# amankhullar/MMBiDAF

Hardware: NVIDIA B200
Metric: mmbidaf_train_videos_per_s (higher is better)
Workload: dtype bf16 tcgen05 BiDAF + tf32 library GEMMs, fp32 accumulate / soft-max / LSTM

## Files before the change

### mmbidaf_b200/csrc/bidaf_bwd_tc.cu

```cuda
#include <stdlib.h>
#include "tc_common.cuh"

namespace mmb {
using namespace tc;
namespace {

constexpr int TY = 32;
constexpr int Y_PART = TY / 8 * GROUP_BYTES;
constexpr int MAX_STAGES = 3;
constexpr int COL_S = 0, COL_GA = 32, COL_GB = 64, COL_ACC0 = 96, COL_ACC1 = 96 + DPAD;
constexpr int STG_STRIDE = 204;
constexpr int NTHREADS = 256;
constexpr int PART_STRIDE = 3 * DPAD;
constexpr float NEG2 = kNegFill * LOG2E;

enum Mode { PT = 0, DC = 1, DQ = 2 };

__device__ __forceinline__ void l2_prefetch(const void* p, size_t bytes) {
  const uintptr_t lo = (reinterpret_cast<uintptr_t>(p) + 15) & ~uintptr_t(15), hi = (reinterpret_cast<uintptr_t>(p) + bytes) & ~uintptr_t(15);
  if (hi > lo) asm volatile("cp.async.bulk.prefetch.L2.global [%0], %1;" ::"l"(lo), "r"((uint32_t)(hi - lo)) : "memory");
}

struct PrepArgs {
  const float* grad;
  const float* text;
  const float* out;
  const float* bm;
  __nv_bfloat16* da_pack;
  __nv_bfloat16* dbm_pack;
  float* d_text;
  float* d_row;
  int L, LP, d;
};

constexpr int PACK_CHUNK_STRIDE = 144;

__device__ __forceinline__ void ld8(const float* p, float* v) {
  const float4 a = __ldg(reinterpret_cast<const float4*>(p)), b = __ldg(reinterpret_cast<const float4*>(p + 4));
  v[0] = a.x; v[1] = a.y; v[2] = a.z; v[3] = a.w; v[4] = b.x; v[5] = b.y; v[6] = b.z; v[7] = b.w;
}

__global__ void __launch_bounds__(256) bidaf_bwd_prep_kernel(const PrepArgs a) {
  __shared__ __align__(16) unsigned char stage[8][CHUNKS * PACK_CHUNK_STRIDE];
  const int b = blockIdx.y, warp = threadIdx.x >> 5, lane = threadIdx.x & 31;
  const int g = blockIdx.x * 8 + warp;
  const int d = a.d, nchunk = d >> 3;
  uint4 da_out[8], dbm_out[8];
#pragma unroll
  for (int r = 0; r < 8; ++r) {
    const int row = g * 8 + r;
    da_out[r] = dbm_out[r] = make_uint4(0u, 0u, 0u, 0u);
    float dot = 0.f;
    const bool on = row < a.L && lane < nchunk;
    if (on) {
      const size_t r4 = ((size_t)b * a.L + row) * 4 * d + lane * 8, r1 = ((size_t)b * a.L + row) * d + lane * 8;
      float g0[8], g1[8], g2[8], g3[8], c[8], av[8], bv[8];
      ld8(a.grad + r4, g0); ld8(a.grad + r4 + d, g1); ld8(a.grad + r4 + 2 * d, g2); ld8(a.grad + r4 + 3 * d, g3);
      ld8(a.text + r1, c); ld8(a.out + r4 + d, av); ld8(a.bm + r1, bv);
      float da[8], db[8], dc[8];
#pragma unroll
      for (int e = 0; e < 8; ++e) {
        da[e] = fmaf(c[e], g2[e], g1[e]);
        db[e] = c[e] * g3[e];
        dc[e] = fmaf(bv[e], g3[e], fmaf(av[e], g2[e], g0[e]));
        dot = fmaf(da[e], av[e], fmaf(db[e], bv[e], dot));
      }
      *reinterpret_cast<float4*>(a.d_text + r1) = make_float4(dc[0], dc[1], dc[2], dc[3]);
      *reinterpret_cast<float4*>(a.d_text + r1 + 4) = make_float4(dc[4], dc[5], dc[6], dc[7]);
      __nv_bfloat162 pa[4], pb[4];
#pragma unroll
      for (int e = 0; e < 4; ++e) {
        pa[e] = __floats2bfloat162_rn(da[2 * e], da[2 * e + 1]);
        pb[e] = __floats2bfloat162_rn(db[2 * e], db[2 * e + 1]);
      }
      da_out[r] = *reinterpret_cast<uint4*>(pa);
      dbm_out[r] = *reinterpret_cast<uint4*>(pb);
    }
    dot = warp_sum(dot);
    if (lane == 0 && row < a.L) a.d_row[(size_t)b * a.L + row] = dot;
  }
  unsigned char* buf = stage[warp];
  const size_t base = ((size_t)b * (a.LP / 8) + g) * GROUP_BYTES;
#pragma unroll 1
  for (int which = 0; which < 2; ++which) {
    if (lane < CHUNKS) {
#pragma unroll
      for (int r = 0; r < 8; ++r)
        *reinterpret_cast<uint4*>(buf + lane * PACK_CHUNK_STRIDE + r * 16) = which == 0 ? da_out[r] : dbm_out[r];
    }
    __syncwarp();
    uint4* dst = reinterpret_cast<uint4*>(reinterpret_cast<char*>(which == 0 ? a.da_pack : a.dbm_pack) + base);
    for (int i = lane; i < CHUNKS * 8; i += 32)
      dst[i] = *reinterpret_cast<const uint4*>(buf + (i >> 3) * PACK_CHUNK_STRIDE + (i & 7) * 16);
    __syncwarp();
  }
}

struct BwdArgs {
  const __nv_bfloat16* x_ops[4];
  const __nv_bfloat16* y_ops[4];
  const unsigned long long* x_words;
  const unsigned long long* y_words;
  const float* bias;
  const float* norm_x;
  const float* norm_y;
  const float* dlt_x;
  const float* dlt_y;
  const float* x_feat;
  const uint8_t* x_keep;
  const float* w_term;
  const float* w_fold;
  const float* t_feat;
  float* dx;
  __nv_bfloat16* dt_pack;
  float* d_col;
  float* part;
  long long* trace;
  float keep_scale;
  int LX, LXP, LY, LYP, d;
  int prefetch;
};

template <int MODE>
__device__ __forceinline__ void bwd_block(const BwdArgs& a, const int b, const int xblk, const int nxb, int* ready,
                                          const int ready_target) {
  constexpr bool IS_PT = MODE == PT;
  constexpr int ROWS = IS_PT ? 128 : 64;
  constexpr int NX = IS_PT ? 1 : 4, NY = IS_PT ? 3 : 4;
  constexpr int X_BYTES = ROWS / 8 * GROUP_BYTES;
  constexpr int TILE_BYTES = ROWS * TY * 2;
  constexpr int TILE_LBO = ROWS * 16;
  constexpr int STAGE_BYTES = NY * Y_PART;
  constexpr int HALF = TY / 2;
  constexpr int STAGES = IS_PT ? 3 : 2;
  extern __shared__ __align__(128) unsigned char smem[];
  unsigned char* Xs = smem;
  unsigned char* Ts = Xs + NX * X_BYTES;
  unsigned char* St = Ts + 2 * TILE_BYTES;
  float* ycol = reinterpret_cast<float*>(St + STAGES * STAGE_BYTES);
  uint64_t* bars = reinterpret_cast<uint64_t*>(ycol + 2 * 3 * TY);
  uint32_t* tmem_slot = reinterpret_cast<uint32_t*>(bars + 2 + 2 * MAX_STAGES);

  const int tid = threadIdx.x, warp = tid >> 5, lane = tid & 31;
  const int half = warp >> 2, wq = warp & 3;
  constexpr int MMA_M = IS_PT ? 128 : 64;
  const int row = IS_PT ? wq * 32 + lane : wq * 16 + (lane & 15);
  const bool owner = IS_PT || lane < 16;
  constexpr int MMA_WARP = IS_PT ? 0 : 2, TMA_WARP = IS_PT ? 1 : 3;
  const int warp_u = uniform_warp_idx();
  const uint32_t leader = elect_one();
  const int x0 = xblk * ROWS;
  if (x0 >= a.LX) return;
  const uint32_t bar_x = smem_u32(bars), bar_mma = smem_u32(bars + 1), bar_full0 = smem_u32(bars + 2);
  const uint32_t bar_free0 = smem_u32(bars + 2 + MAX_STAGES);

  if (tid == 0) {
    mbar_init(bar_x, 1);
    for (int s = 0; s < STAGES; ++s) {
      mbar_init(bar_full0 + 8 * s, 1);
      mbar_init(bar_free0 + 8 * s, 1);
    }
    mbar_init(bar_mma, 1);
    fence_barrier_init();
  }
  if (warp == 0) tmem_alloc(smem_u32(tmem_slot), TMEM_COLS);

  int nty = (a.LY + TY - 1) / TY;
  if (MODE == DC) {
    int last = 0;
    for (int w = lane; w < (a.LY + 63) / 64; w += 32) {
      const unsigned long long open = a.y_words[((size_t)b * (a.LYP / 64) + w) * 2 + 1];
      if (open != 0ull) last = 2 * w + ((open >> 32) != 0ull ? 2 : 1);
    }
#pragma unroll
    for (int o = 16; o > 0; o >>= 1) last = max(last, __shfl_xor_sync(0xffffffffu, last, o));
    if (last > 0) nty = min(nty, last);
  }
  const size_t x_off = ((size_t)b * (a.LXP / 8) + x0 / 8) * GROUP_BYTES;
  const size_t y_batch = (size_t)b * (a.LYP / 8) * GROUP_BYTES;
  if (a.prefetch && tid == 32 * 5) {
    const size_t e0 = ((size_t)b * a.LX + x0) * a.d, ne = (size_t)min(ROWS, a.LX - x0) * a.d;
    if (IS_PT) {
      l2_prefetch(a.t_feat + e0, ne * 4);
    } else {
      l2_prefetch(a.x_feat + e0, ne * 4);
      l2_prefetch(a.dx + e0, ne * 4);
      if (a.x_keep) l2_prefetch(a.x_keep + e0, ne);
    }
  }
  const float log2_lx = log2f((float)a.LX);
  const int yl = tid - (IS_PT ? 0 : 6 * 32);
  float yl_lse = 0.f, yl_d2 = 0.f;
  auto fetch_ycol = [&](int t) {
    const int y = t * TY + yl;
    if ((unsigned)yl < (unsigned)TY && y < a.LY) {
      yl_lse = a.norm_y[(size_t)b * a.LY + y];
      if (!IS_PT) yl_d2 = a.dlt_y[(size_t)b * a.LY + y];
    }
  };
  auto store_ycol = [&](int t) {
    if ((unsigned)yl < (unsigned)TY) {
      float n2 = 0.f, d2 = 0.f, fill = NEG2;
      if (t * TY + yl < a.LY) {
        const bool degenerate = yl_lse < -5e29f;
        n2 = degenerate ? log2_lx : yl_lse * LOG2E;
        fill = degenerate ? 0.f : NEG2;
        d2 = yl_d2;
      }
      float* yc = ycol + (t & 1) * 3 * TY;
      yc[yl] = n2;
      yc[TY + yl] = d2;
      yc[2 * TY + yl] = fill;
    }
  };
  if (!IS_PT && ready) {
    if (tid == 0) wait_counter(ready + b, ready_target);
    __syncthreads();
    fence_proxy_async_all();
  }
  fetch_ycol(0);
  store_ycol(0);
  tc_fence_before();
  __syncthreads();
  tc_fence_after();
  const uint32_t tmem = __shfl_sync(0xffffffffu, *tmem_slot, 0);

  auto issue_stage = [&](int t) {
    const int s = t % STAGES;
    const uint32_t bar = bar_full0 + 8 * s;
    const uint32_t dst = smem_u32(St + s * STAGE_BYTES);
    const size_t off = y_batch + (size_t)t * Y_PART;
    mbar_expect_tx(bar, STAGE_BYTES, leader);
#pragma unroll
    for (int p = 0; p < NY; ++p)
      tma_bulk_g2s(dst + p * Y_PART, reinterpret_cast<const char*>(a.y_ops[p]) + off, Y_PART, bar, leader);
  };
  if (warp_u == TMA_WARP) {
    mbar_expect_tx(bar_x, NX * X_BYTES, leader);
#pragma unroll
    for (int p = 0; p < NX; ++p)
      tma_bulk_g2s(smem_u32(Xs + p * X_BYTES), reinterpret_cast<const char*>(a.x_ops[p]) + x_off, X_BYTES, bar_x, leader);
    for (int t = 0; t < STAGES && t < nty; ++t) issue_stage(t);
  }

  const float bias2 = a.bias[0] * LOG2E;
  const int gx = x0 + row;
  bool valid_x = false, open_x = false;
  float n1 = 0.f, d1 = 0.f;
  if (owner) {
    const ulonglong2 xw = *reinterpret_cast<const ulonglong2*>(a.x_words + ((size_t)b * (a.LXP / 64) + gx / 64) * 2);
    valid_x = (xw.x >> (gx & 63)) & 1ull;
    open_x = (xw.y >> (gx & 63)) & 1ull;
    if (!IS_PT && valid_x) {
      n1 = a.norm_x[(size_t)b * a.LX + gx] * LOG2E;
      d1 = a.dlt_x[(size_t)b * a.LX + gx];
    }
  }
  const uint32_t lane_base = tmem + ((uint32_t)(wq * 32) << 16);
  uint32_t mma_phase = 0;
  float rsum = 0.f;
  constexpr uint32_t IDESC_S = idesc_bf16(TY, 0, MMA_M), IDESC_PV = idesc_bf16(DPAD, 1, MMA_M);
  const uint32_t xs_lo = desc_lo(smem_u32(Xs), 128), ts_lo = desc_lo(smem_u32(Ts), TILE_LBO);

  const bool tracing = a.trace != nullptr && b == 0 && xblk == 0 && tid == MMA_WARP * 32;
  int ntrace = 0;
  auto stamp = [&]() {
    if (tracing && ntrace < 250) a.trace[ntrace++] = clock64();
  };
  stamp();
  if (warp_u == MMA_WARP) mbar_wait(bar_x, 0);
  stamp();
  for (int t = 0; t < nty; ++t) {
    const int s = t % STAGES;
    const uint32_t st_addr = smem_u32(St + s * STAGE_BYTES);
    if (warp_u == MMA_WARP) {
      mbar_wait(bar_full0 + 8 * s, (t / STAGES) & 1);
      stamp();
      tc_fence_after();
      const uint32_t st_lo = desc_lo(st_addr, 128);
      constexpr int NPROD = IS_PT ? 1 : 4;
#pragma unroll
      for (int p = 0; p < NPROD; ++p) {
        const int col = p == 0 ? COL_S : p == 1 ? COL_GA : p == 3 ? COL_GB : (MODE == DC ? COL_GA : COL_GB);
        const bool fresh = p == 0 || p == 1 || (p == 2 && MODE == DQ) || (p == 3 && MODE == DC);
#pragma unroll
        for (int k = 0; k < DPAD / 16; ++k)
          umma_bf16_lh(tmem + col, xs_lo + (p * X_BYTES + k * 256) / 16, desc_hi(GROUP_BYTES),
                       st_lo + (p * Y_PART + k * 256) / 16, desc_hi(GROUP_BYTES), IDESC_S, !(fresh && k == 0), leader);
      }
      umma_commit(bar_mma, leader);
      stamp();
    }
    const ulonglong2 words = *reinterpret_cast<const ulonglong2*>(a.y_words + ((size_t)b * (a.LYP / 64) + (t >> 1)) * 2);
    const int sh = (t & 1) * 32 + half * HALF;
    const uint32_t wvalid = (uint32_t)(words.x >> sh) & 0xffffu, wopen = (uint32_t)(words.y >> sh) & 0xffffu;
    if (t + 1 < nty) fetch_ycol(t + 1);
    if (warp_u == TMA_WARP && t >= 1 && t - 1 + STAGES < nty) {
      mbar_wait(bar_free0 + 8 * ((t - 1) % STAGES), ((t - 1) / STAGES) & 1);
      issue_stage(t - 1 + STAGES);
    }
    mbar_wait(bar_mma, mma_phase);
    mma_phase ^= 1;
    tc_fence_after();
    stamp();

    {
      const float* yc = ycol + (t & 1) * 3 * TY + half * HALF;
      float sv[HALF];
      tmem_ld16(lane_base + COL_S + half * HALF, sv);
      uint32_t pk0[HALF / 2], pk1[HALF / 2];
      if (IS_PT) {
        float n2[HALF];
#pragma unroll
        for (int c = 0; c < HALF; c += 4) *reinterpret_cast<float4*>(n2 + c) = *reinterpret_cast<const float4*>(yc + c);
        const bool masked_row = __any_sync(0xffffffffu, valid_x && !open_x);
#pragma unroll
        for (int c = 0; c < HALF; c += 2) {
          float w[2];
#pragma unroll
          for (int e = 0; e < 2; ++e) {
            float logit = fmaf(sv[c + e], LOG2E, bias2);
            if (masked_row && !open_x) logit = yc[2 * TY + c + e];
            w[e] = (valid_x && ((wvalid >> (c + e)) & 1u)) ? fast_exp2(logit - n2[c + e]) : 0.f;
          }
          const __nv_bfloat162 v = __floats2bfloat162_rn(w[0], w[1]);
          pk0[c / 2] = *reinterpret_cast<const uint32_t*>(&v);
        }
      } else {
        float ga[HALF], gb[HALF], n2[HALF], d2[HALF];
        tmem_ld16(lane_base + COL_GA + half * HALF, ga);
        tmem_ld16(lane_base + COL_GB + half * HALF, gb);
#pragma unroll
        for (int c = 0; c < HALF; c += 4) {
          *reinterpret_cast<float4*>(n2 + c) = *reinterpret_cast<const float4*>(yc + c);
          *reinterpret_cast<float4*>(d2 + c) = *reinterpret_cast<const float4*>(yc + TY + c);
        }
        const bool interior = (wvalid & wopen) == 0xffffu && __all_sync(0xffffffffu, open_x || !valid_x);
        if (interior) {
#pragma unroll
          for (int c = 0; c < HALF; c += 2) {
            float ds[2], rr[2];
#pragma unroll
            for (int e = 0; e < 2; ++e) {
              const float s2 = fmaf(sv[c + e], LOG2E, bias2);
              const float w1 = valid_x ? fast_exp2(s2 - n1) : 0.f, w2 = valid_x ? fast_exp2(s2 - n2[c + e]) : 0.f;
              const float t2 = w2 * (gb[c + e] - d2[c + e]);
              ds[e] = fmaf(w1, ga[c + e] - d1, t2);
              rsum += t2;
              rr[e] = w2;
            }
            const __nv_bfloat162 v = __floats2bfloat162_rn(ds[0], ds[1]);
            pk0[c / 2] = *reinterpret_cast<const uint32_t*>(&v);
            if (MODE == DC) {
              const __nv_bfloat162 r2 = __floats2bfloat162_rn(rr[0], rr[1]);
              pk1[c / 2] = *reinterpret_cast<const uint32_t*>(&r2);
            }
          }
        } else {
#pragma unroll
          for (int c = 0; c < HALF; c += 2) {
            float ds[2], rr[2];
#pragma unroll
            for (int e = 0; e < 2; ++e) {
              const float s2 = fmaf(sv[c + e], LOG2E, bias2);
              const bool vy = (wvalid >> (c + e)) & 1u, oy = (wopen >> (c + e)) & 1u;
              const float w1 = fast_exp2(s2 - n1), w2 = fast_exp2(s2 - n2[c + e]);
              const float t1 = (valid_x && oy) ? w1 * (ga[c + e] - d1) : 0.f;
              const float t2 = (open_x && vy) ? w2 * (gb[c + e] - d2[c + e]) : 0.f;
              ds[e] = t1 + t2;
              rsum += t2;
              if (MODE == DC) rr[e] = (valid_x && vy) ? (open_x ? w2 : fast_exp2(yc[2 * TY + c + e] - n2[c + e])) : 0.f;
            }
            const __nv_bfloat162 v = __floats2bfloat162_rn(ds[0], ds[1]);
            pk0[c / 2] = *reinterpret_cast<const uint32_t*>(&v);
            if (MODE == DC) {
              const __nv_bfloat162 r2 = __floats2bfloat162_rn(rr[0], rr[1]);
              pk1[c / 2] = *reinterpret_cast<const uint32_t*>(&r2);
            }
          }
        }
      }
      unsigned char* trow = Ts + row * 16 + (half * (HALF / 8)) * TILE_LBO;
      if (owner) {
#pragma unroll
        for (int c8 = 0; c8 < HALF / 8; ++c8) {
          *reinterpret_cast<uint4*>(trow + c8 * TILE_LBO) = make_uint4(pk0[c8 * 4], pk0[c8 * 4 + 1], pk0[c8 * 4 + 2], pk0[c8 * 4 + 3]);
          if (MODE == DC)
            *reinterpret_cast<uint4*>(trow + TILE_BYTES + c8 * TILE_LBO) =
                make_uint4(pk1[c8 * 4], pk1[c8 * 4 + 1], pk1[c8 * 4 + 2], pk1[c8 * 4 + 3]);
        }
      }
    }
    if (t + 1 < nty) store_ycol(t + 1);
    fence_proxy_async();
    tc_fence_before();
    __syncthreads();
    stamp();
    if (warp_u == MMA_WARP) {
      tc_fence_after();
      const uint32_t v_lo = desc_lo(st_addr, GROUP_BYTES);
#pragma unroll
      for (int k = 0; k < TY / 16; ++k)
        umma_bf16_lh(tmem + COL_ACC0, ts_lo + k * 2 * TILE_LBO / 16, desc_hi(128),
                     v_lo + ((IS_PT ? 1 : 0) * Y_PART + k * 2 * GROUP_BYTES) / 16, desc_hi(128), IDESC_PV, (t > 0) || (k > 0),
                     leader);
      if (MODE != DQ) {
#pragma unroll
        for (int k = 0; k < TY / 16; ++k)
          umma_bf16_lh(tmem + COL_ACC1, ts_lo + ((IS_PT ? 0 : TILE_BYTES) + k * 2 * TILE_LBO) / 16, desc_hi(128),
                       v_lo + ((IS_PT ? 2 : 3) * Y_PART + k * 2 * GROUP_BYTES) / 16, desc_hi(128), IDESC_PV,
                       (t > 0) || (k > 0), leader);
      }
      umma_commit(t == nty - 1 ? bar_mma : bar_free0 + 8 * s, leader);
    }
  }
  mbar_wait(bar_mma, mma_phase);
  tc_fence_after();
  __syncthreads();
  stamp();

  float* stg = reinterpret_cast<float*>(smem);
  const int d = a.d, dv4 = d >> 2;
  auto drain = [&](int col0, float* dst) {
#pragma unroll 1
    for (int q = half; q < DPAD / 16; q += 2) {
      float o[16];
      tmem_ld16(lane_base + col0 + q * 16, o);
      if (owner) {
#pragma unroll
        for (int i = 0; i < 16; i += 4)
          if (q * 16 + i < STG_STRIDE)
            *reinterpret_cast<float4*>(dst + row * STG_STRIDE + q * 16 + i) = make_float4(o[i], o[i + 1], o[i + 2], o[i + 3]);
      }
    }
  };
  if (IS_PT) {
    drain(COL_ACC0, stg);
    __syncthreads();
    for (int i = tid; i < ROWS * dv4; i += NTHREADS) {
      const int r = i / dv4, c4 = i - r * dv4;
      if (x0 + r < a.LX)
        *reinterpret_cast<float4*>(a.dx + ((size_t)b * a.LX + x0 + r) * d + c4 * 4) =
            *reinterpret_cast<const float4*>(stg + r * STG_STRIDE + c4 * 4);
    }
    __syncthreads();
    drain(COL_ACC1, stg);
    __syncthreads();
    char* tp = reinterpret_cast<char*>(a.dt_pack) + x_off;
    for (int i = tid; i < ROWS * CHUNKS; i += NTHREADS) {
      const int g8 = i / (CHUNKS * 8), rem = i - g8 * CHUNKS * 8, ch = rem >> 3, r8 = rem & 7;
      const int r = g8 * 8 + r8;
      __nv_bfloat162 v[4];
#pragma unroll
      for (int e = 0; e < 4; ++e) {
        const int col = ch * 8 + 2 * e;
        const bool ok = (x0 + r < a.LX) && col < d;
        v[e] = __floats2bfloat162_rn(ok ? stg[r * STG_STRIDE + col] : 0.f, ok ? stg[r * STG_STRIDE + col + 1] : 0.f);
      }
      *reinterpret_cast<uint4*>(tp + (size_t)i * 16) = *reinterpret_cast<uint4*>(v);
    }
    constexpr int NW = NTHREADS / 32, RB = 8;
#pragma unroll 1
    for (int r0 = warp; r0 < ROWS; r0 += NW * RB) {
      float4 tv[RB][2];
#pragma unroll
      for (int u = 0; u < RB; ++u) {
        const int r = r0 + u * NW;
        const float* trow = a.t_feat + ((size_t)b * a.LX + min(x0 + r, a.LX - 1)) * d;
#pragma unroll
        for (int h = 0; h < 2; ++h) {
          const int c4 = lane + 32 * h;
          tv[u][h] = c4 < dv4 ? __ldg(reinterpret_cast<const float4*>(trow + c4 * 4)) : make_float4(0.f, 0.f, 0.f, 0.f);
        }
      }
#pragma unroll
      for (int u = 0; u < RB; ++u) {
        const int r = r0 + u * NW;
        float dot = 0.f;
#pragma unroll
        for (int h = 0; h < 2; ++h) {
          const int c4 = lane + 32 * h;
          if (c4 < dv4) {
            const float4 sv4 = *reinterpret_cast<const float4*>(stg + r * STG_STRIDE + c4 * 4);
            dot += tv[u][h].x * sv4.x + tv[u][h].y * sv4.y + tv[u][h].z * sv4.z + tv[u][h].w * sv4.w;
          }
        }
        dot = warp_sum(dot);
        if (lane == 0 && x0 + r < a.LX) a.d_col[(size_t)b * a.LX + x0 + r] = dot;
      }
    }
  } else {
    float* stg1 = stg + ROWS * STG_STRIDE;
    float* xsum = ycol;
    static_assert(IS_PT || 2 * ROWS <= 2 * 3 * TY, "xsum fits in ycol");
    drain(COL_ACC0, stg);
    if (MODE == DC) drain(COL_ACC1, stg1);
    if (owner) xsum[half * ROWS + row] = rsum;
    __syncthreads();
    const int ngrp = NTHREADS / dv4, rg = tid / dv4, c4 = tid - rg * dv4;
    const int nrow = min(ROWS, a.LX - x0);
    float* red = reinterpret_cast<float*>(St);
    float pt[4] = {0.f, 0.f, 0.f, 0.f}, pf[4] = {0.f, 0.f, 0.f, 0.f}, p_sum = 0.f;
    if (rg < ngrp) {
      float wtv[4], wfv[4];
#pragma unroll
      for (int e = 0; e < 4; ++e) {
        wtv[e] = a.w_term[c4 * 4 + e];
        wfv[e] = a.w_fold ? a.w_fold[c4 * 4 + e] : 1.f;
      }
      constexpr int BATCH = 7;
#pragma unroll 1
      for (int r0 = rg; r0 < nrow; r0 += BATCH * ngrp) {
        float4 xv[BATCH], dv[BATCH];
        uchar4 kv[BATCH];
#pragma unroll
        for (int u = 0; u < BATCH; ++u) {
          const int r = r0 + u * ngrp;
          if (r < nrow) {
            const size_t gi = ((size_t)b * a.LX + x0 + r) * d + c4 * 4;
            xv[u] = __ldg(reinterpret_cast<const float4*>(a.x_feat + gi));
            dv[u] = *reinterpret_cast<const float4*>(a.dx + gi);
            kv[u] = a.x_keep ? __ldg(reinterpret_cast<const uchar4*>(a.x_keep + gi)) : make_uchar4(1, 1, 1, 1);
          }
        }
#pragma unroll
        for (int u = 0; u < BATCH; ++u) {
          const int r = r0 + u * ngrp;
          if (r < nrow) {
            const float rs = xsum[r] + xsum[ROWS + r];
            const float4 v04 = *reinterpret_cast<const float4*>(stg + r * STG_STRIDE + c4 * 4);
            float4 v14 = make_float4(0.f, 0.f, 0.f, 0.f);
            if (MODE == DC) v14 = *reinterpret_cast<const float4*>(stg1 + r * STG_STRIDE + c4 * 4);
            const float x[4] = {xv[u].x, xv[u].y, xv[u].z, xv[u].w}, v0[4] = {v04.x, v04.y, v04.z, v04.w};
            const float v1[4] = {v14.x, v14.y, v14.z, v14.w};
            const unsigned char kk[4] = {kv[u].x, kv[u].y, kv[u].z, kv[u].w};
            float o[4] = {dv[u].x, dv[u].y, dv[u].z, dv[u].w};
#pragma unroll
            for (int e = 0; e < 4; ++e) {
              const float ks = a.x_keep ? (kk[e] ? a.keep_scale : 0.f) : 1.f;
              const float xd = x[e] * ks;
              o[e] += ks * fmaf(rs, wtv[e], v0[e] * wfv[e]) + v1[e];
              pt[e] = fmaf(xd, rs, pt[e]);
              pf[e] = fmaf(xd, v0[e], pf[e]);
            }
            p_sum += rs;
            const size_t gi = ((size_t)b * a.LX + x0 + r) * d + c4 * 4;
            *reinterpret_cast<float4*>(a.dx + gi) = make_float4(o[0], o[1], o[2], o[3]);
          }
        }
      }
      *reinterpret_cast<float4*>(red + (rg * 2 + 0) * d + c4 * 4) = make_float4(pt[0], pt[1], pt[2], pt[3]);
      *reinterpret_cast<float4*>(red + (rg * 2 + 1) * d + c4 * 4) = make_float4(pf[0], pf[1], pf[2], pf[3]);
      if (c4 == 0) red[ngrp * 2 * d + rg] = p_sum;
    }
    __syncthreads();
    if (tid < d) {
      float s_term = 0.f, s_fold = 0.f, s_sum = 0.f;
      for (int g = 0; g < ngrp; ++g) {
        s_term += red[(g * 2 + 0) * d + tid];
        s_fold += red[(g * 2 + 1) * d + tid];
        if (tid == 0) s_sum += red[ngrp * 2 * d + g];
      }
      float* part = a.part + ((size_t)b * nxb + xblk) * PART_STRIDE;
      part[tid] = s_term;
      part[DPAD + tid] = s_fold;
      if (tid == 0) part[2 * DPAD] = s_sum;
    }
  }
  tc_fence_before();
  __syncthreads();
  stamp();
  if (tracing) a.trace[255] = ntrace;
  if (warp == 0) tmem_dealloc(tmem, TMEM_COLS);
  if (IS_PT && ready && tid == 0) signal_counter(ready + b);
}

template <int MODE>
__global__ void __launch_bounds__(NTHREADS, 1) bidaf_bwd_tc_kernel(const BwdArgs a) {
  bwd_block<MODE>(a, blockIdx.y, blockIdx.x, gridDim.x, nullptr, 0);
}

struct BwdFusedArgs {
  BwdArgs k[3];
  int* ready;
  int n_pt, n_dc, n_dq;
  int nb[3];
  int dq_first;
};

__global__ void __launch_bounds__(NTHREADS, 1) bidaf_bwd_fused_kernel(const BwdFusedArgs f) {
  const int blk = blockIdx.x;
  if (blk < f.n_pt) {
    bwd_block<PT>(f.k[PT], blk / f.nb[PT], blk % f.nb[PT], f.nb[PT], f.ready, 0);
    return;
  }
  int i = blk - f.n_pt;
  bool is_dq;
  if (f.dq_first) {
    is_dq = i < f.n_dq;
    if (!is_dq) i -= f.n_dq;
  } else {
    is_dq = i >= f.n_dc;
    if (is_dq) i -= f.n_dc;
  }
  if (is_dq) bwd_block<DQ>(f.k[DQ], i / f.nb[DQ], i % f.nb[DQ], f.nb[DQ], f.ready, f.nb[PT]);
  else bwd_block<DC>(f.k[DC], i / f.nb[DC], i % f.nb[DC], f.nb[DC], f.ready, f.nb[PT]);
}

template <int MODE>
constexpr size_t bwd_smem_bytes() {
  constexpr int ROWS = MODE == PT ? 128 : 64;
  constexpr int NX = MODE == PT ? 1 : 4, NY = MODE == PT ? 3 : 4;
  constexpr int STAGES = MODE == PT ? 3 : 2;
  return (size_t)NX * (ROWS / 8 * GROUP_BYTES) + 2 * (ROWS * TY * 2) + (size_t)STAGES * NY * Y_PART + 2 * 3 * TY * 4 +
         (2 + 2 * MAX_STAGES) * 8 + 16;
}

struct ReduceArgs {
  const float* part_c;
  const float* part_q;
  float *d_w_text, *d_w_cross, *d_w_modality, *d_bias;
  int B, gx_c, nb_c, gx_q, nb_q, d;
};

constexpr int RED_COLS = 16;

__global__ void __launch_bounds__(256) bidaf_bwd_reduce_kernel(const ReduceArgs a) {
  __shared__ float red[256];
  const int nblk = (a.d + RED_COLS - 1) / RED_COLS;
  const int which = blockIdx.x / nblk;
  const int tid = threadIdx.x;
  float acc = 0.f;
  if (which < 3) {
    const int k = (blockIdx.x - which * nblk) * RED_COLS + (tid & (RED_COLS - 1)), grp = tid / RED_COLS;
    const float* part = which == 2 ? a.part_q : a.part_c;
    const int gx = which == 2 ? a.gx_q : a.gx_c, nb = which == 2 ? a.nb_q : a.nb_c;
    const int off = which == 1 ? DPAD : 0;
    if (k < a.d)
      for (int i = grp; i < a.B * nb; i += 256 / RED_COLS) {
        const int b = i / nb, xb = i - b * nb;
        acc += part[((size_t)b * gx + xb) * PART_STRIDE + off + k];
      }
    red[tid] = acc;
    __syncthreads();
    if (grp == 0 && k < a.d) {
      float s = 0.f;
      for (int g = 0; g < 256 / RED_COLS; ++g) s += red[g * RED_COLS + tid];
      (which == 0 ? a.d_w_text : which == 1 ? a.d_w_cross : a.d_w_modality)[k] = s;
    }
  } else {
    for (int i = tid; i < a.B * a.nb_c; i += 256) {
      const int b = i / a.nb_c, xb = i - b * a.nb_c;
      acc += a.part_c[((size_t)b * a.gx_c + xb) * PART_STRIDE + 2 * DPAD];
    }
    red[tid] = acc;
    __syncthreads();
    for (int s = 128; s > 0; s >>= 1) {
      if (tid < s) red[tid] += red[tid + s];
      __syncthreads();
    }
    if (tid == 0) a.d_bias[0] = red[0];
  }
}

struct BwdWorkspace {
  __nv_bfloat16 *da_pack, *dbm_pack, *dt_pack;
  float *d_row, *d_col, *part_c, *part_q;
  int* ready;
  long long* trace;
  size_t bytes;
};
BwdWorkspace bwd_workspace(void* workspace, int B, int Lc, int Lq) {
  const BidafPacks pk = bidaf_packs(nullptr, B, Lc, Lq, false);
  char* ws = static_cast<char*>(workspace);
  BwdWorkspace w;
  size_t off = 0;
  auto take = [&](size_t bytes) {
    char* p = ws + off;
    off += (bytes + 255) / 256 * 256;
    return p;
  };
  w.da_pack = reinterpret_cast<__nv_bfloat16*>(take(pk.c_pack));
  w.dbm_pack = reinterpret_cast<__nv_bfloat16*>(take(pk.c_pack));
  w.dt_pack = reinterpret_cast<__nv_bfloat16*>(take(pk.q_pack));
  w.d_row = reinterpret_cast<float*>(take((size_t)B * Lc * 4));
  w.d_col = reinterpret_cast<float*>(take((size_t)B * Lq * 4));
  w.part_c = reinterpret_cast<float*>(take((size_t)B * (pk.LcP / 64) * PART_STRIDE * 4));
  w.part_q = reinterpret_cast<float*>(take((size_t)B * (pk.LqP / 64) * PART_STRIDE * 4));
  w.ready = reinterpret_cast<int*>(take((size_t)B * 4));
  w.trace = reinterpret_cast<long long*>(take(3 * 256 * 8));
  w.bytes = off;
  return w;
}

}

size_t bidaf_bwd_tc_workspace_bytes(int B, int Lc, int Lq) { return bwd_workspace(nullptr, B, Lc, Lq).bytes; }

int bidaf_bwd_tc(const float* grad_out, const float* text, const float* modality, const float* w_text,
                 const float* w_modality, const float* w_cross, const float* bias, const uint8_t* keep_text,
                 const uint8_t* keep_modality, float keep_scale, const float* out, const float* bm, const float* q2c,
                 const float* lse_row, const float* lse_col, const void* fwd_workspace, void* workspace, float* d_text,
                 float* d_modality, float* d_w_text, float* d_w_modality, float* d_w_cross, float* d_bias, int B, int Lc,
                 int Lq, int d, cudaStream_t stream) {
  MMB_REQUIRE(d % 8 == 0 && d <= 200, MMB_ERR_UNSUPPORTED, "mmb_bidaf_bwd (bf16 tier): d=%d (need d %% 8 == 0, d <= 200)", d);
  MMB_REQUIRE(fwd_workspace && workspace, MMB_ERR_INVALID, "mmb_bidaf_bwd (bf16 tier): workspace is null");
  const BidafPacks pk = bidaf_packs(const_cast<void*>(fwd_workspace), B, Lc, Lq, keep_modality != nullptr);
  const BwdWorkspace w = bwd_workspace(workspace, B, Lc, Lq);
  const int LcP = pk.LcP, LqP = pk.LqP;
  const char* env = getenv("MMB_BIDAF_BWD_STAGES");
  const int stages = env ? atoi(env) : 31;
  const bool tracing = getenv("MMB_BIDAF_BWD_TRACE") != nullptr;

  if (stages & 1) {
  PrepArgs pa{grad_out, text, out, bm, w.da_pack, w.dbm_pack, d_text, w.d_row, Lc, LcP, d};
  bidaf_bwd_prep_kernel<<<dim3(LcP / 64, B), 256, 0, stream>>>(pa);
  if (int rc = check_launch("bidaf_bwd_prep_kernel")) return rc;
  }
  BwdArgs pt{}, dc{}, dq{};
  {
    BwdArgs& a = pt;
    a.x_ops[0] = pk.qs;
    a.y_ops[0] = pk.cw; a.y_ops[1] = w.da_pack; a.y_ops[2] = w.dbm_pack;
    a.x_words = pk.q_words; a.y_words = pk.c_words; a.bias = bias;
    a.norm_y = lse_row;
    a.t_feat = q2c; a.dx = d_modality; a.dt_pack = w.dt_pack; a.d_col = w.d_col;
    a.LX = Lq; a.LXP = LqP; a.LY = Lc; a.LYP = LcP; a.d = d;
    a.trace = tracing ? w.trace : nullptr;
  }
  {
    BwdArgs& a = dc;
    a.x_ops[0] = pk.cw; a.x_ops[1] = w.da_pack; a.x_ops[2] = w.dbm_pack; a.x_ops[3] = pk.cp;
    a.y_ops[0] = pk.qs; a.y_ops[1] = pk.qp; a.y_ops[2] = pk.tp; a.y_ops[3] = w.dt_pack;
    a.x_words = pk.c_words; a.y_words = pk.q_words; a.bias = bias;
    a.norm_x = lse_row; a.norm_y = lse_col; a.dlt_x = w.d_row; a.dlt_y = w.d_col;
    a.x_feat = text; a.x_keep = keep_text; a.w_term = w_text; a.w_fold = w_cross;
    a.dx = d_text; a.part = w.part_c; a.keep_scale = keep_scale;
    a.LX = Lc; a.LXP = LcP; a.LY = Lq; a.LYP = LqP; a.d = d;
    a.trace = tracing ? w.trace + 256 : nullptr;
  }
  {
    BwdArgs& a = dq;
    a.x_ops[0] = pk.qs; a.x_ops[1] = w.dt_pack; a.x_ops[2] = pk.qp; a.x_ops[3] = pk.tp;
    a.y_ops[0] = pk.cw; a.y_ops[1] = pk.cp; a.y_ops[2] = w.da_pack; a.y_ops[3] = w.dbm_pack;
    a.x_words = pk.q_words; a.y_words = pk.c_words; a.bias = bias;
    a.norm_x = lse_col; a.norm_y = lse_row; a.dlt_x = w.d_col; a.dlt_y = w.d_row;
    a.x_feat = modality; a.x_keep = keep_modality; a.w_term = w_modality; a.w_fold = nullptr;
    a.dx = d_modality; a.part = w.part_q; a.keep_scale = keep_scale;
    a.LX = Lq; a.LXP = LqP; a.LY = Lc; a.LYP = LcP; a.d = d;
    a.trace = tracing ? w.trace + 512 : nullptr;
  }
  static const char* pf_env = getenv("MMB_BIDAF_BWD_PREFETCH");
  pt.prefetch = dc.prefetch = dq.prefetch = pf_env ? atoi(pf_env) : 1;
  constexpr size_t smem_pt = bwd_smem_bytes<PT>(), smem_dc = bwd_smem_bytes<DC>(), smem_dq = bwd_smem_bytes<DQ>();
  static_assert(smem_dc <= 227 * 1024 && smem_dq <= 227 * 1024 && smem_pt <= 227 * 1024, "shared memory");
  if (!env) {
    constexpr size_t smem = smem_dc > smem_pt ? (smem_dc > smem_dq ? smem_dc : smem_dq) : (smem_pt > smem_dq ? smem_pt : smem_dq);
    static const char* ord_env = getenv("MMB_BIDAF_BWD_ORDER");
    const int dq_first = ord_env ? atoi(ord_env) : (Lc >= Lq ? 1 : 0);
    BwdFusedArgs f{{pt, dc, dq}, w.ready, B * (LqP / 128), B * (LcP / 64), B * (LqP / 64), {LqP / 128, LcP / 64, LqP / 64}, dq_first};
    MMB_CUDA(cudaMemsetAsync(w.ready, 0, sizeof(int) * (size_t)B, stream));
    MMB_CUDA(cudaFuncSetAttribute(bidaf_bwd_fused_kernel, cudaFuncAttributeMaxDynamicSharedMemorySize, (int)smem));
    bidaf_bwd_fused_kernel<<<f.n_pt + f.n_dc + f.n_dq, NTHREADS, smem, stream>>>(f);
    if (int rc = check_launch("bidaf_bwd_fused_kernel")) return rc;
  } else {
    if (stages & 2) {
      MMB_CUDA(cudaFuncSetAttribute(bidaf_bwd_tc_kernel<PT>, cudaFuncAttributeMaxDynamicSharedMemorySize, (int)smem_pt));
      bidaf_bwd_tc_kernel<PT><<<dim3(LqP / 128, B), NTHREADS, smem_pt, stream>>>(pt);
      if (int rc = check_launch("bidaf_bwd_tc_kernel<PT>")) return rc;
    }
    if (stages & 4) {
      MMB_CUDA(cudaFuncSetAttribute(bidaf_bwd_tc_kernel<DC>, cudaFuncAttributeMaxDynamicSharedMemorySize, (int)smem_dc));
      bidaf_bwd_tc_kernel<DC><<<dim3(LcP / 64, B), NTHREADS, smem_dc, stream>>>(dc);
      if (int rc = check_launch("bidaf_bwd_tc_kernel<DC>")) return rc;
    }
    if (stages & 8) {
      MMB_CUDA(cudaFuncSetAttribute(bidaf_bwd_tc_kernel<DQ>, cudaFuncAttributeMaxDynamicSharedMemorySize, (int)smem_dq));
      bidaf_bwd_tc_kernel<DQ><<<dim3(LqP / 64, B), NTHREADS, smem_dq, stream>>>(dq);
      if (int rc = check_launch("bidaf_bwd_tc_kernel<DQ>")) return rc;
    }
  }
  if (!(stages & 16)) return MMB_OK;
  ReduceArgs ra{w.part_c, w.part_q, d_w_text, d_w_cross, d_w_modality, d_bias, B, LcP / 64, (Lc + 63) / 64, LqP / 64,
                (Lq + 63) / 64, d};
  bidaf_bwd_reduce_kernel<<<3 * ((d + RED_COLS - 1) / RED_COLS) + 1, 256, 0, stream>>>(ra);
  return check_launch("bidaf_bwd_reduce_kernel");
}

}
```

### mmbidaf_b200/csrc/bidaf_fwd_tc5.cu

```cuda
#include <stdlib.h>
#include "tc_common.cuh"

namespace mmb {
using namespace tc;
namespace {

constexpr int TX = 128, TY = 64;
constexpr int X_BYTES = TX / 8 * GROUP_BYTES;
constexpr int SLOT_BYTES = TY / 8 * GROUP_BYTES;
constexpr int NSLOT = 4;
constexpr int STG_STRIDE = 116;
constexpr int STG_BYTES = TX * STG_STRIDE * 4;
constexpr int NSOFT = 4, NEPI = 4;
constexpr int EPI_WARP0 = 4, MMA_WARP = 8, TMA_WARP = 9, XLOAD_WARP = 10, NTHREADS = 12 * 32;
constexpr int N_LO = 112, N_HI = DPAD - N_LO;
constexpr int COL_S = 0, COL_P = 2 * TY, COL_LO = COL_P + TY, COL_HI = COL_LO + 2 * N_LO;
static_assert(COL_HI + N_HI == TMEM_COLS, "TMEM budget");
constexpr int ITEM_SLOTS = 4;
constexpr int N_CONSUMERS = NSOFT + NEPI + 2;
constexpr float TAU2 = 11.0f;
constexpr float NEG2 = kNegFill * LOG2E;

enum Kind { PQ = 0, PA = 1, PB = 2, DONE = 3 };

struct PassArgs {
  const __nv_bfloat16* s_pack;
  const __nv_bfloat16* v_pack;
  const unsigned long long* y_words;
  int LX, LXP, LY, LYP;
};

struct Args {
  PassArgs p[3];
  const __nv_bfloat16* x_pack[3];
  const __nv_bfloat16* c_pack;
  float* out;
  float* q2c;
  float* bm;
  __nv_bfloat16* t_pack;
  float* lse_row;
  float* lse_col;
  const float* bias;
  int* ready;
  int* queue;
  int nq, nc, n_q2c, n_c2q, d;
  long long* trace;
  long long* ev;
  int dbg;
};

struct EvLog {
  long long* p;
  int n;
  __device__ __forceinline__ void operator()(int code) {
    if (p && n < 1024) {
      p[2 * n] = code;
      p[2 * n + 1] = clock64();
      ++n;
    }
  }
};

__device__ __forceinline__ void mbar_arrive(uint32_t bar) {
  asm volatile("mbarrier.arrive.shared::cta.b64 _, [%0];" ::"r"(bar) : "memory");
}
__device__ __forceinline__ void named_bar_sync(int id, int nthreads) {
  asm volatile("bar.sync %0, %1;" ::"r"(id), "r"(nthreads) : "memory");
}
__device__ __forceinline__ void tmem_ld16_nowait(uint32_t taddr, uint32_t* r) {
  asm volatile(
      "tcgen05.ld.sync.aligned.32x32b.x16.b32 {%0,%1,%2,%3,%4,%5,%6,%7,%8,%9,%10,%11,%12,%13,%14,%15}, [%16];"
      : "=r"(r[0]), "=r"(r[1]), "=r"(r[2]), "=r"(r[3]), "=r"(r[4]), "=r"(r[5]), "=r"(r[6]), "=r"(r[7]), "=r"(r[8]),
        "=r"(r[9]), "=r"(r[10]), "=r"(r[11]), "=r"(r[12]), "=r"(r[13]), "=r"(r[14]), "=r"(r[15])
      : "r"(taddr)
      : "memory");
}
__device__ __forceinline__ void tmem_st16_u32(uint32_t taddr, const uint32_t* v) {
  asm volatile(
      "tcgen05.st.sync.aligned.32x32b.x16.b32 [%0], {%1,%2,%3,%4,%5,%6,%7,%8,%9,%10,%11,%12,%13,%14,%15,%16};" ::"r"(taddr),
      "r"(v[0]), "r"(v[1]), "r"(v[2]), "r"(v[3]), "r"(v[4]), "r"(v[5]), "r"(v[6]), "r"(v[7]), "r"(v[8]), "r"(v[9]), "r"(v[10]),
      "r"(v[11]), "r"(v[12]), "r"(v[13]), "r"(v[14]), "r"(v[15])
      : "memory");
}
__device__ __forceinline__ void umma_bf16_ts(uint32_t d_tmem, uint32_t a_tmem, uint32_t b_lo, uint32_t b_hi, uint32_t idesc,
                                             uint32_t acc, uint32_t leader) {
  asm volatile(
      "{\n\t"
      ".reg .pred p, q;\n\t"
      ".reg .b64 db;\n\t"
      "setp.ne.b32 p, %5, 0;\n\t"
      "setp.ne.b32 q, %6, 0;\n\t"
      "mov.b64 db, {%2, %3};\n\t"
      "@q tcgen05.mma.cta_group::1.kind::f16 [%0], [%1], db, %4, p;\n\t"
      "}" ::"r"(d_tmem), "r"(a_tmem), "r"(b_lo), "r"(b_hi), "r"(idesc), "r"(acc), "r"(leader)
      : "memory");
}
__device__ __forceinline__ void st_cs_f4(float* p, const float4 v) {
  asm volatile("st.global.cs.v4.f32 [%0], {%1, %2, %3, %4};" ::"l"(p), "f"(v.x), "f"(v.y), "f"(v.z), "f"(v.w) : "memory");
}
__device__ __forceinline__ int4 ld_item(const int4* p) {
  int4 v;
  asm volatile("ld.shared.v4.s32 {%0, %1, %2, %3}, [%4];" : "=r"(v.x), "=r"(v.y), "=r"(v.z), "=r"(v.w) : "r"(smem_u32(p)) : "memory");
  return v;
}
__device__ __forceinline__ void signal_release(int* counter) {
  asm volatile("red.release.gpu.global.add.s32 [%0], 1;" ::"l"(counter) : "memory");
}

constexpr int NBARS = 2 * ITEM_SLOTS + 2 + 2 * NSLOT + 4 * 2 + 2 + 2 + 1 + 2 + 2;
constexpr size_t SMEM_BYTES = (size_t)X_BYTES + NSLOT * SLOT_BYTES + STG_BYTES + 2 * TX * 4 + ITEM_SLOTS * 16 + NBARS * 8 + 16;
static_assert(SMEM_BYTES <= 227 * 1024, "one CTA per SM");


__device__ __noinline__ void stage_fill(float* stg_row, const uint32_t acc, const int ch0, const int nch, const float inv_l) {
#pragma unroll 1
  for (int c = 0; c < nch; ++c) {
    uint32_t raw[16];
    tmem_ld16_nowait(acc + (ch0 + c) * 16, raw);
    tmem_wait_ld();
#pragma unroll
    for (int i = 0; i < 16; i += 4)
      *reinterpret_cast<float4*>(stg_row + (ch0 + c) * 16 + i) =
          make_float4(__uint_as_float(raw[i]) * inv_l, __uint_as_float(raw[i + 1]) * inv_l, __uint_as_float(raw[i + 2]) * inv_l,
                      __uint_as_float(raw[i + 3]) * inv_l);
  }
}

__device__ __forceinline__ void load_c16(uint2* cv, const char* c, const int cnt) {
#pragma unroll
  for (int j = 0; j < 16; ++j) {
    cv[j] = make_uint2(0u, 0u);
    if (j < cnt) cv[j] = __ldg(reinterpret_cast<const uint2*>(c + (j >> 1) * GROUP_BYTES + (j & 1) * 64));
  }
}
__device__ __forceinline__ float4 bf16x4_to_float4(const uint2 v) {
  return make_float4(__uint_as_float(v.x << 16), __uint_as_float(v.x & 0xffff0000u), __uint_as_float(v.y << 16),
                     __uint_as_float(v.y & 0xffff0000u));
}
__device__ __forceinline__ void st_f4_if(float* p, const float4 v, const uint32_t plain, const uint32_t streaming) {
  asm volatile(
      "{\n\t"
      ".reg .pred a, b;\n\t"
      "setp.ne.u32 a, %5, 0;\n\t"
      "setp.ne.u32 b, %6, 0;\n\t"
      "@a st.global.v4.f32 [%0], {%1, %2, %3, %4};\n\t"
      "@b st.global.cs.v4.f32 [%0], {%1, %2, %3, %4};\n\t"
      "}" ::"l"(p), "f"(v.x), "f"(v.y), "f"(v.z), "f"(v.w), "r"(plain), "r"(streaming)
      : "memory");
}
__device__ __forceinline__ void store16(const uint2* cv, const float* sp, float* pa, float* pb, const uint32_t a8, const uint32_t b8,
                                        const int cnt, const uint32_t a_plain, const uint32_t a_cs, const uint32_t b_on) {
#pragma unroll
  for (int j = 0; j < 16; ++j) {
    if (j < cnt) {
      const float4 o = *reinterpret_cast<const float4*>(sp + j * (NEPI * STG_STRIDE));
      st_f4_if(pa, o, a_plain, a_cs);
      const float4 c = bf16x4_to_float4(cv[j]);
      st_f4_if(pb, make_float4(c.x * o.x, c.y * o.y, c.z * o.z, c.w * o.w), 0u, b_on);
    }
    pa += a8;
    pb += b8;
  }
}

__device__ __noinline__ void write_t_pack(char* tp_block, const float* stg, const int e, const int lane, const int col0, const int ncols,
                                          const int rows, const int d) {
  const int r8 = lane & 7, cq = lane >> 3;
  const int nch = ncols / 8, chunk0 = col0 / 8;
#pragma unroll 1
  for (int rg = e; rg < TX / 8; rg += NEPI) {
    const int row = rg * 8 + r8;
    char* dst = tp_block + (size_t)rg * GROUP_BYTES + r8 * 16;
    const float* src = stg + row * STG_STRIDE;
#pragma unroll 1
    for (int ch = cq; ch < nch; ch += 4) {
      const float4 lo = *reinterpret_cast<const float4*>(src + ch * 8), hi = *reinterpret_cast<const float4*>(src + ch * 8 + 4);
      const bool ok = row < rows && (chunk0 + ch) * 8 < d;
      __nv_bfloat162 h[4];
      h[0] = __floats2bfloat162_rn(ok ? lo.x : 0.f, ok ? lo.y : 0.f);
      h[1] = __floats2bfloat162_rn(ok ? lo.z : 0.f, ok ? lo.w : 0.f);
      h[2] = __floats2bfloat162_rn(ok ? hi.x : 0.f, ok ? hi.y : 0.f);
      h[3] = __floats2bfloat162_rn(ok ? hi.z : 0.f, ok ? hi.w : 0.f);
      *reinterpret_cast<uint4*>(dst + (chunk0 + ch) * 128) = *reinterpret_cast<uint4*>(h);
    }
  }
}

__global__ void __launch_bounds__(NTHREADS, 1) bidaf_tc5_kernel(const Args f) {
  extern __shared__ __align__(128) unsigned char smem_raw[];
  unsigned char* const sX = smem_raw;
  unsigned char* const sY = sX + X_BYTES;
  float* const sStage = reinterpret_cast<float*>(sY + NSLOT * SLOT_BYTES);
  float* const sStat = reinterpret_cast<float*>(reinterpret_cast<unsigned char*>(sStage) + STG_BYTES);
  int4* const sItems = reinterpret_cast<int4*>(sStat + 2 * TX);
  uint64_t* const sBars = reinterpret_cast<uint64_t*>(sItems + ITEM_SLOTS);
  uint32_t* const sTmem = reinterpret_cast<uint32_t*>(sBars + NBARS);

  const int tid = threadIdx.x, lane = tid & 31;
  const int warp_u = uniform_warp_idx();
  const uint32_t leader = elect_one();

  const uint32_t b0 = smem_u32(sBars);
  const uint32_t item_full0 = b0, item_empty0 = item_full0 + 8 * ITEM_SLOTS;
  const uint32_t x_full = item_empty0 + 8 * ITEM_SLOTS, x_free = x_full + 8;
  const uint32_t slot_full0 = x_free + 8, slot_free0 = slot_full0 + 8 * NSLOT;
  const uint32_t s_full0 = slot_free0 + 8 * NSLOT, s_free0 = s_full0 + 16;
  const uint32_t p_full0 = s_free0 + 16, p_free0 = p_full0 + 16;
  const uint32_t o_full0 = p_free0 + 16, lo_free0 = o_full0 + 16, hi_free = lo_free0 + 16;
  const uint32_t st_full0 = hi_free + 8, st_free0 = st_full0 + 16;

  if (tid == 0) {
    for (int i = 0; i < ITEM_SLOTS; ++i) {
      mbar_init(item_full0 + 8 * i, 1);
      mbar_init(item_empty0 + 8 * i, N_CONSUMERS);
    }
    mbar_init(x_full, 1);
    mbar_init(x_free, 1);
    for (int i = 0; i < NSLOT; ++i) {
      mbar_init(slot_full0 + 8 * i, 1);
      mbar_init(slot_free0 + 8 * i, 1);
    }
    for (int i = 0; i < 2; ++i) {
      mbar_init(s_full0 + 8 * i, 1);
      mbar_init(s_free0 + 8 * i, NSOFT);
      mbar_init(p_full0 + 8 * i, NSOFT);
      mbar_init(p_free0 + 8 * i, 1);
      mbar_init(o_full0 + 8 * i, 1);
      mbar_init(lo_free0 + 8 * i, 1);
      mbar_init(st_full0 + 8 * i, NSOFT);
      mbar_init(st_free0 + 8 * i, NEPI);
    }
    mbar_init(hi_free, 1);
    fence_barrier_init();
  }
  if (warp_u == 0) tmem_alloc(smem_u32(sTmem), TMEM_COLS);
  tc_fence_before();
  __syncthreads();
  tc_fence_after();
  const uint32_t tmem = *reinterpret_cast<volatile uint32_t*>(sTmem);
  const int n_items = f.n_q2c + 2 * f.n_c2q;

  if (warp_u == TMA_WARP) {
    asm volatile("griddepcontrol.wait;" ::: "memory");
    uint32_t g = 0;
    EvLog ev{(f.ev && blockIdx.x == 0 && lane == 0) ? f.ev + 2 * 2048 : nullptr, 0};
    for (uint32_t n = 0;; ++n) {
      int item = 0;
      if (leader) item = atomicAdd(f.queue, 1);
      item = __shfl_sync(0xffffffffu, item, __ffs(__ballot_sync(0xffffffffu, leader)) - 1);
      int kind = DONE, b = 0, xblk = 0, nty = 0, canon = 0;
      if (item < n_items) {
        const int n1 = f.n_q2c + f.n_c2q;
        if (item < n1) {
          const int qb = (int)((long long)item * f.n_q2c / n1), qa = (int)((long long)(item + 1) * f.n_q2c / n1);
          if (qa > qb) { kind = PQ; b = qb / f.nq; xblk = qb - b * f.nq; canon = qb; }
          else { kind = PA; const int i = item - qb; b = i / f.nc; xblk = i - b * f.nc; canon = f.n_q2c + i; }
        } else {
          kind = PB;
          const int i = item - n1;
          b = i / f.nc;
          xblk = i - b * f.nc;
          canon = item;
        }
        const PassArgs& a = f.p[kind];
        nty = (a.LY + TY - 1) / TY;
        int last = 0;
        for (int w = lane; w < nty; w += 32)
          if (a.y_words[((size_t)b * (a.LYP / 64) + w) * 2 + 1] != 0ull) last = w + 1;
#pragma unroll
        for (int o = 16; o > 0; o >>= 1) last = max(last, __shfl_xor_sync(0xffffffffu, last, o));
        if (last > 0) nty = min(nty, last);
      }
      const int slot = n & (ITEM_SLOTS - 1);
      mbar_wait(item_empty0 + 8 * slot, ((n / ITEM_SLOTS) & 1) ^ 1);
      if (lane == 0) {
        sItems[slot] = make_int4(kind, b, xblk, nty);
        if (f.trace && kind != DONE) {
          long long* tr = f.trace + (size_t)canon * 8;
          tr[0] = globaltimer_ns();
          tr[3] = kind;
          tr[5] = nty;
        }
      }
      __syncwarp();
      if (lane == 0) mbar_arrive(item_full0 + 8 * slot);
      ev(kind);
      if (kind == DONE) break;
      const PassArgs& a = f.p[kind];
      const size_t y_batch = (size_t)b * (a.LYP / 8) * GROUP_BYTES;
      if (kind == PB) {
        wait_counter(f.ready + b, f.nq * NEPI);
        fence_proxy_async_all();
      }
      const bool same_v = a.v_pack == a.s_pack;
#pragma unroll 1
      for (int t = 0; t < nty; ++t) {
        const size_t off = y_batch + (size_t)t * SLOT_BYTES;
#pragma unroll 1
        for (int part = 0; part < (same_v ? 1 : 2); ++part, ++g) {
          const int s = g % NSLOT;
          mbar_wait(slot_free0 + 8 * s, ((g / NSLOT) & 1) ^ 1);
          if (part == 0) ev(100 + t);
          mbar_expect_tx(slot_full0 + 8 * s, SLOT_BYTES, leader);
          tma_bulk_g2s(smem_u32(sY + s * SLOT_BYTES), reinterpret_cast<const char*>(part == 0 ? a.s_pack : a.v_pack) + off, SLOT_BYTES,
                       slot_full0 + 8 * s, leader);
        }
      }
    }
  } else if (warp_u == MMA_WARP) {
    constexpr uint32_t IDESC_S = idesc_bf16(TY, 0), IDESC_LO = idesc_bf16(N_LO, 1), IDESC_HI = idesc_bf16(N_HI, 1);
    uint32_t g = 0;
    uint32_t gt = 0;
    uint32_t nx = 0;
    const uint32_t xs_lo = desc_lo(smem_u32(sX), 128);
    EvLog ev{(f.ev && blockIdx.x == 0 && lane == 0) ? f.ev : nullptr, 0};
    for (uint32_t n = 0;; ++n) {
      const int slot = n & (ITEM_SLOTS - 1);
      mbar_wait(item_full0 + 8 * slot, (n / ITEM_SLOTS) & 1);
      const int4 it = ld_item(sItems + slot);
      __syncwarp();
      if (lane == 0) mbar_arrive(item_empty0 + 8 * slot);
      const int kind = it.x, nty = it.w;
      if (kind == DONE) break;
      const bool same_v = f.p[kind].v_pack == f.p[kind].s_pack;
      const uint32_t per = same_v ? 1u : 2u;
      const int ob = n & 1;
      ev(kind);
      mbar_wait(x_full, nx & 1);
      ++nx;
      ev(10);
      tc_fence_after();
      if (f.trace && lane == 0)
        f.trace[(size_t)(kind == PQ ? it.y * f.nq + it.z : f.n_q2c + f.n_c2q * (kind == PB ? 1 : 0) + it.y * f.nc + it.z) * 8 + 7] = globaltimer_ns();
      auto issue_s = [&](int t) {
        const uint32_t gg = g + per * t, tt = gt + t;
        const int s = gg % NSLOT, sb = tt & 1;
        mbar_wait(slot_full0 + 8 * s, (gg / NSLOT) & 1);
        ev(200 + t);
        mbar_wait(s_free0 + 8 * sb, ((tt >> 1) & 1) ^ 1);
        ev(300 + t);
        tc_fence_after();
        const uint32_t y_lo = desc_lo(smem_u32(sY + s * SLOT_BYTES), 128);
#pragma unroll
        for (int k = 0; k < DPAD / 16; ++k)
          umma_bf16_lh(tmem + COL_S + sb * TY, xs_lo + k * 16, desc_hi(GROUP_BYTES), y_lo + k * 16, desc_hi(GROUP_BYTES), IDESC_S,
                       k > 0, leader);
        umma_commit(s_full0 + 8 * sb, leader);
        if (!same_v) umma_commit(slot_free0 + 8 * s, leader);
        if (t == nty - 1) umma_commit(x_free, leader);
      };
      int s_issued = 0;
      for (int t = 0; t < nty; ++t) {
        while (s_issued < nty && s_issued < t + 2) issue_s(s_issued++);
        const uint32_t gg = g + per * t + (per - 1), tt = gt + t;
        const int s = gg % NSLOT, pb = tt & 1;
        if (t == 0) {
          mbar_wait(lo_free0 + 8 * ob, ((n >> 1) & 1) ^ 1);
          mbar_wait(hi_free, (n & 1) ^ 1);
        }
        if (!same_v) mbar_wait(slot_full0 + 8 * s, (gg / NSLOT) & 1);
        mbar_wait(p_full0 + 8 * pb, (tt >> 1) & 1);
        ev(400 + t);
        tc_fence_after();
        const uint32_t v_lo = desc_lo(smem_u32(sY + s * SLOT_BYTES), GROUP_BYTES);
        const uint32_t p_addr = tmem + COL_P + pb * (TY / 2);
#pragma unroll
        for (int k = 0; k < TY / 16; ++k) {
          const uint32_t acc = (t > 0) || (k > 0);
          umma_bf16_ts(tmem + COL_LO + ob * N_LO, p_addr + k * 8, v_lo + k * (2 * GROUP_BYTES / 16), desc_hi(128), IDESC_LO, acc, leader);
          umma_bf16_ts(tmem + COL_HI, p_addr + k * 8, v_lo + k * (2 * GROUP_BYTES / 16) + (N_LO / 8) * (128 / 16), desc_hi(128), IDESC_HI,
                       acc, leader);
        }
        umma_commit(slot_free0 + 8 * s, leader);
        umma_commit(p_free0 + 8 * pb, leader);
        if (t == nty - 1) umma_commit(o_full0 + 8 * ob, leader);
      }
      g += per * nty;
      gt += nty;
    }
  } else if (warp_u == XLOAD_WARP) {
    uint32_t nx = 0;
    for (uint32_t n = 0;; ++n) {
      const int slot = n & (ITEM_SLOTS - 1);
      mbar_wait(item_full0 + 8 * slot, (n / ITEM_SLOTS) & 1);
      const int4 it = ld_item(sItems + slot);
      __syncwarp();
      if (lane == 0) mbar_arrive(item_empty0 + 8 * slot);
      if (it.x == DONE) break;
      const PassArgs& a = f.p[it.x];
      const size_t x_off = ((size_t)it.y * (a.LXP / 8) + (size_t)it.z * (TX / 8)) * GROUP_BYTES;
      mbar_wait(x_free, (nx & 1) ^ 1);
      ++nx;
      mbar_expect_tx(x_full, X_BYTES, leader);
      tma_bulk_g2s(smem_u32(sX), reinterpret_cast<const char*>(f.x_pack[it.x]) + x_off, X_BYTES, x_full, leader);
    }
  } else if (warp_u < NSOFT) {
    const int row = warp_u * 32 + lane;
    const uint32_t lane_base = tmem + ((uint32_t)(warp_u * 32) << 16);
    const float bias2 = f.bias[0] * LOG2E;
    uint32_t gt = 0;
    EvLog ev{(f.ev && blockIdx.x == 0 && tid == 0) ? f.ev + 2048 : nullptr, 0};
    for (uint32_t n = 0;; ++n) {
      const int slot = n & (ITEM_SLOTS - 1);
      mbar_wait(item_full0 + 8 * slot, (n / ITEM_SLOTS) & 1);
      const int4 it = ld_item(sItems + slot);
      __syncwarp();
      if (lane == 0) mbar_arrive(item_empty0 + 8 * slot);
      const int kind = it.x, b = it.y, xblk = it.z, nty = it.w;
      if (kind == DONE) break;
      const PassArgs& a = f.p[kind];
      const int ob = n & 1;
      const unsigned long long* words_b = a.y_words + (size_t)b * (a.LYP / 64) * 2;
      float m_ref = -INFINITY, l_run = 0.f;
      ulonglong2 words = *reinterpret_cast<const ulonglong2*>(words_b);
#pragma unroll 1
      for (int t = 0; t < nty; ++t, ++gt) {
        const int sb = gt & 1;
        const uint32_t sk = (gt >> 1) & 1;
        const unsigned long long wvalid = words.x, wopen = words.y;
        const bool all_open = (wvalid & wopen) == ~0ull;
        if (t + 1 < nty) words = *reinterpret_cast<const ulonglong2*>(words_b + (size_t)(t + 1) * 2);
        mbar_wait(s_full0 + 8 * sb, sk);
        ev(200 + t);
        tc_fence_after();
        const uint32_t s_addr = lane_base + COL_S + sb * TY;
        float tile_max = -INFINITY;
#pragma unroll 1
        for (int h = 0; h < 2; ++h) {
          uint32_t raw[32];
          tmem_ld16_nowait(s_addr + h * 32, raw);
          tmem_ld16_nowait(s_addr + h * 32 + 16, raw + 16);
          tmem_wait_ld();
          float mx[4] = {-INFINITY, -INFINITY, -INFINITY, -INFINITY};
          if (all_open) {
#pragma unroll
            for (int c = 0; c < 32; ++c) mx[c & 3] = fmaxf(mx[c & 3], __uint_as_float(raw[c]));
          } else {
            const uint32_t wv = (uint32_t)(wvalid >> (32 * h)), wo = (uint32_t)(wopen >> (32 * h));
#pragma unroll
            for (int c = 0; c < 32; ++c) {
              const float v = ((wo >> c) & 1u) ? fmaf(__uint_as_float(raw[c]), LOG2E, bias2) : NEG2;
              if ((wv >> c) & 1u) mx[c & 3] = fmaxf(mx[c & 3], v);
            }
          }
          tile_max = fmaxf(tile_max, fmaxf(fmaxf(mx[0], mx[1]), fmaxf(mx[2], mx[3])));
        }
        if (all_open) tile_max = fmaf(tile_max, LOG2E, bias2);
        float alpha = 1.f;
        const bool bump = tile_max > m_ref + TAU2;
        if (bump) {
          alpha = fast_exp2(m_ref - tile_max);
          m_ref = tile_max;
        }
        const float shift = bias2 - m_ref;
        ev(400 + t);
        mbar_wait(p_free0 + 8 * sb, sk ^ 1);
        ev(500 + t);
        tc_fence_after();
        float psum = 0.f;
#pragma unroll 1
        for (int h = 0; h < 2; ++h) {
          uint32_t raw[32];
          tmem_ld16_nowait(s_addr + h * 32, raw);
          tmem_ld16_nowait(s_addr + h * 32 + 16, raw + 16);
          tmem_wait_ld();
          if (h == 1) {
            tc_fence_before();
            __syncwarp();
            if (lane == 0) mbar_arrive(s_free0 + 8 * sb);
          }
          uint32_t packed[16];
          float ps[2] = {0.f, 0.f};
          if (all_open) {
#pragma unroll
            for (int c = 0; c < 32; c += 2) {
              const float p0 = fast_exp2(fmaf(__uint_as_float(raw[c]), LOG2E, shift));
              const float p1 = fast_exp2(fmaf(__uint_as_float(raw[c + 1]), LOG2E, shift));
              ps[0] += p0;
              ps[1] += p1;
              const __nv_bfloat162 pk = __floats2bfloat162_rn(p0, p1);
              packed[c / 2] = *reinterpret_cast<const uint32_t*>(&pk);
            }
          } else {
            const uint32_t wv = (uint32_t)(wvalid >> (32 * h)), wo = (uint32_t)(wopen >> (32 * h));
#pragma unroll
            for (int c = 0; c < 32; c += 2) {
              const float s0 = ((wo >> c) & 1u) ? fmaf(__uint_as_float(raw[c]), LOG2E, bias2) : NEG2;
              const float s1 = ((wo >> (c + 1)) & 1u) ? fmaf(__uint_as_float(raw[c + 1]), LOG2E, bias2) : NEG2;
              const float p0 = ((wv >> c) & 1u) ? fast_exp2(s0 - m_ref) : 0.f;
              const float p1 = ((wv >> (c + 1)) & 1u) ? fast_exp2(s1 - m_ref) : 0.f;
              ps[0] += p0;
              ps[1] += p1;
              const __nv_bfloat162 pk = __floats2bfloat162_rn(p0, p1);
              packed[c / 2] = *reinterpret_cast<const uint32_t*>(&pk);
            }
          }
          psum += ps[0] + ps[1];
          tmem_st16_u32(lane_base + COL_P + sb * (TY / 2) + h * 16, packed);
        }
        l_run = l_run * alpha + psum;
        if (__any_sync(0xffffffffu, bump && t > 0)) {
          mbar_wait(p_free0 + 8 * (sb ^ 1), ((gt - 1) >> 1) & 1);
          tc_fence_after();
#pragma unroll 1
          for (int q = 0; q < DPAD / 16; ++q) {
            const uint32_t addr = lane_base + (q < N_LO / 16 ? COL_LO + ob * N_LO + q * 16 : COL_HI + (q - N_LO / 16) * 16);
            float o[16];
            tmem_ld16(addr, o);
#pragma unroll
            for (int i = 0; i < 16; ++i) o[i] *= alpha;
            tmem_st16(addr, o);
          }
        }
        tmem_wait_st();
        tc_fence_before();
        __syncwarp();
        if (lane == 0) mbar_arrive(p_full0 + 8 * sb);
        ev(600 + t);
      }
      mbar_wait(st_free0 + 8 * ob, ((n >> 1) & 1) ^ 1);
      sStat[ob * TX + row] = l_run;
      __syncwarp();
      if (lane == 0) mbar_arrive(st_full0 + 8 * ob);
      float* lse = kind == PQ ? f.lse_col : (kind == PA ? f.lse_row : nullptr);
      if (lse && xblk * TX + row < a.LX) lse[(size_t)b * a.LX + xblk * TX + row] = (m_ref + log2f(l_run)) * LN2;
    }
  } else if (warp_u < EPI_WARP0 + NEPI) {
    const int e = warp_u - EPI_WARP0, q4 = e & 3;
    const uint32_t lane_base = tmem + ((uint32_t)(q4 * 32) << 16);
    float* const stg_row = sStage + (q4 * 32 + lane) * STG_STRIDE;
    EvLog ev{(f.ev && blockIdx.x == 0 && e == (f.dbg >> 8) && lane == 0) ? f.ev + 3 * 2048 : nullptr, 0};
    for (uint32_t n = 0;; ++n) {
      const int slot = n & (ITEM_SLOTS - 1);
      mbar_wait(item_full0 + 8 * slot, (n / ITEM_SLOTS) & 1);
      const int4 it = ld_item(sItems + slot);
      __syncwarp();
      if (lane == 0) mbar_arrive(item_empty0 + 8 * slot);
      const int kind = it.x, b = it.y, xblk = it.z;
      if (kind == DONE) break;
      ev(20 + kind);
      const int ob = n & 1;
      const uint32_t par = (n >> 1) & 1;
      const int x0 = xblk * TX, LX = f.p[kind].LX, d = f.d;
      const size_t row0 = (size_t)b * LX + x0;
      const int rows = min(TX, LX - x0);
      const int cnt = rows > e ? (rows - e + NEPI - 1) / NEPI : 0;
      const int cnt0 = min(cnt, 16), cnt1 = max(cnt - 16, 0);
      const uint32_t d8 = NEPI * d;
      const char* c_row = reinterpret_cast<const char*>(f.c_pack) + ((size_t)b * (f.p[PA].LXP / 8) + (size_t)(x0 / 8)) * GROUP_BYTES + e * 16 +
                          (lane >> 1) * 128 + (lane & 1) * 8;
      float* const pa_base = kind == PA ? f.out + d : (kind == PB ? f.bm : f.q2c);
      float* pa_row = (pa_base ? pa_base : f.out) + (row0 + e) * (kind == PA ? 4 * d : d) + 4 * lane;
      float* pb_row = f.out + (row0 + e) * 4 * d + (kind == PA ? 2 : 3) * d + 4 * lane;
      const uint32_t a8 = kind == PA ? 4 * d8 : d8, b8 = 4 * d8;
      const bool dbg_st = (f.dbg & 2) != 0;
      const uint32_t a_plain = (kind != PA && pa_base && !dbg_st) ? 1u : 0u, a_cs = (kind == PA && !dbg_st) ? 1u : 0u;
      const uint32_t b_on = (kind != PQ && !dbg_st) ? 1u : 0u;
      char* const tp_block = reinterpret_cast<char*>(f.t_pack) + ((size_t)b * (f.p[PQ].LXP / 8) + (size_t)(x0 / 8)) * GROUP_BYTES;
      const int n4_hi = max(0, min(N_HI, d - N_LO)) >> 2, n4_lo = min(N_LO, d) >> 2;
      const float* const sp = sStage + e * STG_STRIDE + 4 * lane;
      const bool ld_hi = lane < n4_hi && kind != PQ && !(f.dbg & 1), ld_lo = lane < n4_lo && kind != PQ && !(f.dbg & 1);
      uint2 cva[16], cvb[16];
      load_c16(cva, c_row + (N_LO / 8) * 128, ld_hi ? cnt0 : 0);
      mbar_wait(st_full0 + 8 * ob, par);
      const float inv_l = 1.f / sStat[ob * TX + q4 * 32 + lane];
      __syncwarp();
      if (lane == 0) mbar_arrive(st_free0 + 8 * ob);
      mbar_wait(o_full0 + 8 * ob, par);
      tc_fence_after();
      long long t_acc = 0;
      if (f.trace && e == 0 && lane == 0) t_acc = globaltimer_ns();
      ev(31);
#pragma unroll 1
      for (int phase = 0; phase < 2; ++phase) {
        const int col0 = phase == 0 ? N_LO : 0, ncols = phase == 0 ? N_HI : N_LO, n4 = phase == 0 ? n4_hi : n4_lo;
        if (!(f.dbg & 8)) stage_fill(stg_row, lane_base + (phase == 0 ? COL_HI : COL_LO + ob * N_LO), 0, ncols / 16, inv_l);
        tc_fence_before();
        named_bar_sync(1, NEPI * 32);
        if (e == 0 && lane == 0) mbar_arrive(phase == 0 ? hi_free : lo_free0 + 8 * ob);
        ev(33 + 4 * phase);
        const bool st = lane < n4, ld = phase == 0 ? ld_hi : ld_lo;
        const int w0 = st ? cnt0 : 0, w1 = st ? cnt1 : 0;
        load_c16(cvb, c_row + (col0 / 8) * 128 + 8 * GROUP_BYTES, ld ? cnt1 : 0);
        if (kind == PQ && !(f.dbg & 8)) write_t_pack(tp_block, sStage, e, lane, col0, ncols, rows, d);
        store16(cva, sp, pa_row + col0, pb_row + col0, a8, b8, w0, a_plain, a_cs, b_on);
        if (phase == 0) load_c16(cva, c_row, ld_lo ? cnt0 : 0);
        store16(cvb, sp + 16 * NEPI * STG_STRIDE, pa_row + col0 + 16 * a8, pb_row + col0 + 16 * b8, a8, b8, w1, a_plain, a_cs, b_on);
        ev(34 + 4 * phase);
        named_bar_sync(1, NEPI * 32);
      }
      if (kind == PQ) {
        __syncwarp();
        if (lane == 0) signal_release(f.ready + b);
      }
      if (f.trace && e == 0 && lane == 0) {
        long long* tr = f.trace + (size_t)(kind == PQ ? b * f.nq + xblk : f.n_q2c + f.n_c2q * (kind == PB ? 1 : 0) + b * f.nc + xblk) * 8;
        tr[1] = t_acc;
        tr[2] = globaltimer_ns();
        uint32_t smid;
        asm volatile("mov.u32 %0, %%smid;" : "=r"(smid));
        tr[4] = smid;
      }
    }
  }
  tc_fence_before();
  __syncthreads();
  if (warp_u == 0) tmem_dealloc(tmem, TMEM_COLS);
}

}

int bidaf_fwd_tc5_launch(const BidafPacks& pk, const float* text, const float* bias, float* out, float* q2c, float* bm,
                         float* lse_row, float* lse_col, int B, int Lc, int Lq, int d, cudaStream_t stream) {
  static_assert(PACK_ROWS == TX, "pack padding must match the X tile");
  const int LcP = pk.LcP, LqP = pk.LqP;
  Args f{};
  f.p[PQ] = PassArgs{pk.cw, pk.cp, pk.c_words, Lq, LqP, Lc, LcP};
  f.p[PA] = PassArgs{pk.qs, pk.qp, pk.q_words, Lc, LcP, Lq, LqP};
  f.p[PB] = PassArgs{pk.qs, pk.tp, pk.q_words, Lc, LcP, Lq, LqP};
  f.x_pack[PQ] = pk.qs;
  f.x_pack[PA] = pk.cw;
  f.x_pack[PB] = pk.cw;
  f.c_pack = pk.cp;
  (void)text;
  f.out = out;
  f.q2c = q2c;
  f.bm = bm;
  f.t_pack = pk.tp;
  f.lse_row = lse_row;
  f.lse_col = lse_col;
  f.bias = bias;
  f.ready = pk.ready;
  f.queue = pk.ready + B;
  f.nq = LqP / TX;
  f.nc = LcP / TX;
  f.n_q2c = B * f.nq;
  f.n_c2q = B * f.nc;
  f.d = d;
  static const char* trace_env = getenv("MMB_BIDAF_FWD_ITEM_TRACE");
  f.trace = trace_env ? reinterpret_cast<long long*>(strtoull(trace_env, nullptr, 0)) : nullptr;
  static const char* ev_env = getenv("MMB_BIDAF_FWD_EV_TRACE");
  f.ev = ev_env ? reinterpret_cast<long long*>(strtoull(ev_env, nullptr, 0)) : nullptr;
  static const char* dbg_env = getenv("MMB_TC5_DEBUG");
  f.dbg = dbg_env ? atoi(dbg_env) : 0;
  static int num_sms = 0;
  if (num_sms == 0) {
    int dev = 0;
    MMB_CUDA(cudaGetDevice(&dev));
    MMB_CUDA(cudaDeviceGetAttribute(&num_sms, cudaDevAttrMultiProcessorCount, dev));
    MMB_CUDA(cudaFuncSetAttribute(bidaf_tc5_kernel, cudaFuncAttributeMaxDynamicSharedMemorySize, (int)SMEM_BYTES));
  }
  const int n_items = f.n_q2c + 2 * f.n_c2q;
  cudaLaunchConfig_t cfg{};
  cfg.gridDim = dim3((unsigned)(n_items < num_sms ? n_items : num_sms));
  cfg.blockDim = dim3(NTHREADS);
  cfg.dynamicSmemBytes = SMEM_BYTES;
  cfg.stream = stream;
  cudaLaunchAttribute attr[1];
  attr[0].id = cudaLaunchAttributeProgrammaticStreamSerialization;
  attr[0].val.programmaticStreamSerializationAllowed = 1;
  cfg.attrs = attr;
  cfg.numAttrs = 1;
  MMB_CUDA(cudaLaunchKernelEx(&cfg, bidaf_tc5_kernel, f));
  return check_launch("bidaf_tc5_kernel");
}

}
```

### mmbidaf_b200/csrc/tc_common.cuh

```cuda
#pragma once
#include <cuda_bf16.h>
#include "common.cuh"

namespace mmb {
namespace tc {

constexpr int DPAD = 208;
constexpr int CHUNKS = DPAD / 8;
constexpr int GROUP_BYTES = CHUNKS * 128;
constexpr int TMEM_COLS = 512;
constexpr float LOG2E = 1.4426950408889634f, LN2 = 0.6931471805599453f;

__device__ __forceinline__ uint32_t smem_u32(const void* p) { return static_cast<uint32_t>(__cvta_generic_to_shared(p)); }

__device__ __forceinline__ uint32_t elect_one() {
  uint32_t pred;
  asm volatile(
      "{\n\t"
      ".reg .pred p;\n\t"
      "elect.sync _|p, 0xffffffff;\n\t"
      "selp.u32 %0, 1, 0, p;\n\t"
      "}"
      : "=r"(pred));
  return pred;
}
__device__ __forceinline__ int uniform_warp_idx() { return __shfl_sync(0xffffffffu, (int)(threadIdx.x >> 5), 0); }

__device__ __forceinline__ void mbar_init(uint32_t bar, uint32_t count) {
  asm volatile("mbarrier.init.shared::cta.b64 [%0], %1;" ::"r"(bar), "r"(count) : "memory");
}
__device__ __forceinline__ void mbar_expect_tx(uint32_t bar, uint32_t bytes, uint32_t leader) {
  asm volatile(
      "{\n\t"
      ".reg .pred q;\n\t"
      "setp.ne.b32 q, %2, 0;\n\t"
      "@q mbarrier.arrive.expect_tx.shared::cta.b64 _, [%0], %1;\n\t"
      "}" ::"r"(bar), "r"(bytes), "r"(leader)
      : "memory");
}
__device__ __forceinline__ void mbar_wait(uint32_t bar, uint32_t parity) {
#pragma unroll 1
  for (uint32_t spin = 0; spin < (1u << 26); ++spin) {
    uint32_t done;
    asm volatile(
        "{\n\t"
        ".reg .pred p;\n\t"
        "mbarrier.try_wait.parity.shared::cta.b64 p, [%1], %2;\n\t"
        "selp.u32 %0, 1, 0, p;\n\t"
        "}"
        : "=r"(done)
        : "r"(bar), "r"(parity)
        : "memory");
    if (done) return;
  }
  __trap();
}
__device__ __forceinline__ void tma_bulk_g2s(uint32_t dst, const void* src, uint32_t bytes, uint32_t bar, uint32_t leader) {
  asm volatile(
      "{\n\t"
      ".reg .pred q;\n\t"
      "setp.ne.b32 q, %4, 0;\n\t"
      "@q cp.async.bulk.shared::cluster.global.mbarrier::complete_tx::bytes [%0], [%1], %2, [%3];\n\t"
      "}" ::"r"(dst), "l"(src), "r"(bytes), "r"(bar), "r"(leader)
      : "memory");
}
__device__ __forceinline__ void fence_proxy_async() { asm volatile("fence.proxy.async.shared::cta;" ::: "memory"); }
__device__ __forceinline__ long long globaltimer_ns() {
  long long t;
  asm volatile("mov.u64 %0, %%globaltimer;" : "=l"(t));
  return t;
}
__device__ __forceinline__ void fence_proxy_async_all() { asm volatile("fence.proxy.async;" ::: "memory"); }
__device__ __forceinline__ void signal_counter(int* counter) {
  __threadfence();
  asm volatile("red.release.gpu.global.add.s32 [%0], 1;" ::"l"(counter) : "memory");
}
__device__ __forceinline__ void wait_counter(const int* counter, int target) {
#pragma unroll 1
  for (uint32_t spin = 0; spin < (1u << 24); ++spin) {
    int v;
    asm volatile("ld.acquire.gpu.global.s32 %0, [%1];" : "=r"(v) : "l"(counter) : "memory");
    if (v >= target) return;
    __nanosleep(64);
  }
  __trap();
}
__device__ __forceinline__ void fence_barrier_init() { asm volatile("fence.mbarrier_init.release.cluster;" ::: "memory"); }
__device__ __forceinline__ void tc_fence_before() { asm volatile("tcgen05.fence::before_thread_sync;" ::: "memory"); }
__device__ __forceinline__ void tc_fence_after() { asm volatile("tcgen05.fence::after_thread_sync;" ::: "memory"); }

__device__ __forceinline__ void tmem_alloc(uint32_t dst_smem, uint32_t cols) {
  asm volatile("tcgen05.alloc.cta_group::1.sync.aligned.shared::cta.b32 [%0], %1;" ::"r"(dst_smem), "r"(cols) : "memory");
  asm volatile("tcgen05.relinquish_alloc_permit.cta_group::1.sync.aligned;" ::: "memory");
}
__device__ __forceinline__ void tmem_dealloc(uint32_t taddr, uint32_t cols) {
  asm volatile("tcgen05.dealloc.cta_group::1.sync.aligned.b32 %0, %1;" ::"r"(taddr), "r"(cols) : "memory");
}
__device__ __forceinline__ void umma_bf16_lh(uint32_t d_tmem, uint32_t a_lo, uint32_t a_hi, uint32_t b_lo, uint32_t b_hi,
                                             uint32_t idesc, uint32_t acc, uint32_t leader) {
  asm volatile(
      "{\n\t"
      ".reg .pred p, q;\n\t"
      ".reg .b64 da, db;\n\t"
      "setp.ne.b32 p, %6, 0;\n\t"
      "setp.ne.b32 q, %7, 0;\n\t"
      "mov.b64 da, {%1, %2};\n\t"
      "mov.b64 db, {%3, %4};\n\t"
      "@q tcgen05.mma.cta_group::1.kind::f16 [%0], da, db, %5, p;\n\t"
      "}" ::"r"(d_tmem), "r"(a_lo), "r"(a_hi), "r"(b_lo), "r"(b_hi), "r"(idesc), "r"(acc), "r"(leader)
      : "memory");
}
__device__ __forceinline__ uint32_t desc_lo(uint32_t addr, uint32_t lbo_bytes) { return ((addr & 0x3FFFFu) >> 4) | ((lbo_bytes >> 4) << 16); }
constexpr uint32_t desc_hi(uint32_t sbo_bytes) { return (sbo_bytes >> 4) | (1u << 14); }
__device__ __forceinline__ void umma_commit(uint32_t bar, uint32_t leader) {
  asm volatile(
      "{\n\t"
      ".reg .pred q;\n\t"
      "setp.ne.b32 q, %1, 0;\n\t"
      "@q tcgen05.commit.cta_group::1.mbarrier::arrive::one.shared::cluster.b64 [%0];\n\t"
      "}" ::"r"(bar), "r"(leader)
      : "memory");
}
__device__ __forceinline__ void tmem_wait_ld() { asm volatile("tcgen05.wait::ld.sync.aligned;" ::: "memory"); }
__device__ __forceinline__ void tmem_wait_st() { asm volatile("tcgen05.wait::st.sync.aligned;" ::: "memory"); }

__device__ __forceinline__ void tmem_ld16(uint32_t taddr, float* v) {
  uint32_t r[16];
  asm volatile(
      "tcgen05.ld.sync.aligned.32x32b.x16.b32 {%0,%1,%2,%3,%4,%5,%6,%7,%8,%9,%10,%11,%12,%13,%14,%15}, [%16];"
      : "=r"(r[0]), "=r"(r[1]), "=r"(r[2]), "=r"(r[3]), "=r"(r[4]), "=r"(r[5]), "=r"(r[6]), "=r"(r[7]), "=r"(r[8]),
        "=r"(r[9]), "=r"(r[10]), "=r"(r[11]), "=r"(r[12]), "=r"(r[13]), "=r"(r[14]), "=r"(r[15])
      : "r"(taddr)
      : "memory");
  tmem_wait_ld();
#pragma unroll
  for (int i = 0; i < 16; ++i) v[i] = __uint_as_float(r[i]);
}
__device__ __forceinline__ void tmem_st16(uint32_t taddr, const float* v) {
  asm volatile(
      "tcgen05.st.sync.aligned.32x32b.x16.b32 [%0], {%1,%2,%3,%4,%5,%6,%7,%8,%9,%10,%11,%12,%13,%14,%15,%16};" ::"r"(taddr),
      "r"(__float_as_uint(v[0])), "r"(__float_as_uint(v[1])), "r"(__float_as_uint(v[2])), "r"(__float_as_uint(v[3])),
      "r"(__float_as_uint(v[4])), "r"(__float_as_uint(v[5])), "r"(__float_as_uint(v[6])), "r"(__float_as_uint(v[7])),
      "r"(__float_as_uint(v[8])), "r"(__float_as_uint(v[9])), "r"(__float_as_uint(v[10])), "r"(__float_as_uint(v[11])),
      "r"(__float_as_uint(v[12])), "r"(__float_as_uint(v[13])), "r"(__float_as_uint(v[14])), "r"(__float_as_uint(v[15]))
      : "memory");
}

constexpr uint32_t idesc_bf16(int n, int b_mn_major, int m = 128) {
  return (1u << 4) | (1u << 7) | (1u << 10) | ((uint32_t)b_mn_major << 16) | ((uint32_t)(n >> 3) << 17) | ((uint32_t)(m >> 4) << 24);
}

__device__ __forceinline__ float fast_exp2(float x) {
  float y;
  asm("ex2.approx.ftz.f32 %0, %1;" : "=f"(y) : "f"(x));
  return y;
}

inline int round_up(int v, int m) { return (v + m - 1) / m * m; }

constexpr int PACK_ROWS = 128;
struct BidafPacks {
  __nv_bfloat16 *cw, *cp;
  __nv_bfloat16 *qs, *qp;
  __nv_bfloat16* tp;
  unsigned long long *c_words, *q_words;
  int* ready;
  int LcP, LqP;
  size_t c_pack, q_pack, bytes;
};
inline BidafPacks bidaf_packs(void* workspace, int B, int Lc, int Lq, bool modality_dropout) {
  BidafPacks p;
  p.LcP = round_up(Lc, PACK_ROWS);
  p.LqP = round_up(Lq, PACK_ROWS);
  p.c_pack = (size_t)B * (p.LcP / 8) * GROUP_BYTES;
  p.q_pack = (size_t)B * (p.LqP / 8) * GROUP_BYTES;
  char* ws = static_cast<char*>(workspace);
  p.cw = reinterpret_cast<__nv_bfloat16*>(ws);
  p.cp = reinterpret_cast<__nv_bfloat16*>(ws + p.c_pack);
  p.qs = reinterpret_cast<__nv_bfloat16*>(ws + 2 * p.c_pack);
  p.tp = reinterpret_cast<__nv_bfloat16*>(ws + 2 * p.c_pack + p.q_pack);
  char* next = ws + 2 * p.c_pack + 2 * p.q_pack;
  p.qp = p.qs;
  if (modality_dropout) {
    p.qp = reinterpret_cast<__nv_bfloat16*>(next);
    next += p.q_pack;
  }
  p.c_words = reinterpret_cast<unsigned long long*>(next);
  p.q_words = p.c_words + (size_t)B * (p.LcP / 64) * 2;
  const size_t used = ((size_t)(next - ws) + 16 * (size_t)B * (p.LcP / 64 + p.LqP / 64) + 255) / 256 * 256;
  p.ready = reinterpret_cast<int*>(ws + used);
  p.bytes = used + ((size_t)(B + 1) * 4 + 255) / 256 * 256;
  return p;
}

}
}
```

Measured before the change: 7508.

## Warp-specialize BiDAF backward kernel with dedicated MMA/TMA warps and split-stage mbarrier pipeline

New measurement: 7602 (median of 6 runs). +1.2%, better.

```diff
diff --git a/mmbidaf_b200/csrc/bidaf_bwd_tc.cu b/mmbidaf_b200/csrc/bidaf_bwd_tc.cu
--- a/mmbidaf_b200/csrc/bidaf_bwd_tc.cu
+++ b/mmbidaf_b200/csrc/bidaf_bwd_tc.cu
@@ -11,6 +11,8 @@
 constexpr int COL_S = 0, COL_GA = 32, COL_GB = 64, COL_ACC0 = 96, COL_ACC1 = 96 + DPAD;
 constexpr int STG_STRIDE = 204;
 constexpr int NTHREADS = 256;
+constexpr int MMA_WARP = 8, TMA_WARP = 9, CTA_THREADS = NTHREADS + 64;
+constexpr int NBARS = 7 + 4 * MAX_STAGES;
 constexpr int PART_STRIDE = 3 * DPAD;
 constexpr float NEG2 = kNegFill * LOG2E;
 
@@ -118,7 +120,6 @@
   long long* trace;
   float keep_scale;
   int LX, LXP, LY, LYP, d;
-  int prefetch;
 };
 
 template <int MODE>
@@ -130,37 +131,51 @@
   constexpr int X_BYTES = ROWS / 8 * GROUP_BYTES;
   constexpr int TILE_BYTES = ROWS * TY * 2;
   constexpr int TILE_LBO = ROWS * 16;
+  constexpr int NT = MODE == DC ? 2 : 1;
   constexpr int STAGE_BYTES = NY * Y_PART;
   constexpr int HALF = TY / 2;
   constexpr int STAGES = IS_PT ? 3 : 2;
+  constexpr uint32_t LATE = IS_PT ? 0x6u : MODE == DC ? 0x9u : 0x1u;
+  constexpr int NPROD = IS_PT ? 1 : 4;
+  constexpr int N_LATE = __builtin_popcount(LATE);
   extern __shared__ __align__(128) unsigned char smem[];
   unsigned char* Xs = smem;
   unsigned char* Ts = Xs + NX * X_BYTES;
-  unsigned char* St = Ts + 2 * TILE_BYTES;
+  unsigned char* St = Ts + 2 * NT * TILE_BYTES;
   float* ycol = reinterpret_cast<float*>(St + STAGES * STAGE_BYTES);
   uint64_t* bars = reinterpret_cast<uint64_t*>(ycol + 2 * 3 * TY);
-  uint32_t* tmem_slot = reinterpret_cast<uint32_t*>(bars + 2 + 2 * MAX_STAGES);
+  uint32_t* tmem_slot = reinterpret_cast<uint32_t*>(bars + NBARS);
 
   const int tid = threadIdx.x, warp = tid >> 5, lane = tid & 31;
-  const int half = warp >> 2, wq = warp & 3;
+  const int half = (warp >> 2) & 1, wq = warp & 3;
   constexpr int MMA_M = IS_PT ? 128 : 64;
   const int row = IS_PT ? wq * 32 + lane : wq * 16 + (lane & 15);
-  const bool owner = IS_PT || lane < 16;
-  constexpr int MMA_WARP = IS_PT ? 0 : 2, TMA_WARP = IS_PT ? 1 : 3;
+  const bool ew = tid < NTHREADS;
+  const bool owner = ew && (IS_PT || lane < 16);
   const int warp_u = uniform_warp_idx();
   const uint32_t leader = elect_one();
   const int x0 = xblk * ROWS;
   if (x0 >= a.LX) return;
-  const uint32_t bar_x = smem_u32(bars), bar_mma = smem_u32(bars + 1), bar_full0 = smem_u32(bars + 2);
-  const uint32_t bar_free0 = smem_u32(bars + 2 + MAX_STAGES);
+  const uint32_t bar_x = smem_u32(bars), bar_s_full = smem_u32(bars + 1), bar_s_empty = smem_u32(bars + 2);
+  const uint32_t bar_done = smem_u32(bars + 3), bar_ts_full0 = smem_u32(bars + 4);
+  const uint32_t bar_rows = smem_u32(bars + 6);
+  const uint32_t full_e0 = smem_u32(bars + 7), full_l0 = full_e0 + 8 * MAX_STAGES;
+  const uint32_t free_e0 = full_l0 + 8 * MAX_STAGES, free_l0 = free_e0 + 8 * MAX_STAGES;
 
   if (tid == 0) {
     mbar_init(bar_x, 1);
+    mbar_init(bar_s_full, 1);
+    mbar_init(bar_s_empty, NTHREADS / 32);
+    mbar_init(bar_done, 1);
+    mbar_init(bar_rows, 1);
+    mbar_init(bar_ts_full0, 1);
+    mbar_init(bar_ts_full0 + 8, 1);
     for (int s = 0; s < STAGES; ++s) {
-      mbar_init(bar_full0 + 8 * s, 1);
-      mbar_init(bar_free0 + 8 * s, 1);
-    }
-    mbar_init(bar_mma, 1);
+      mbar_init(full_e0 + 8 * s, 1);
+      mbar_init(full_l0 + 8 * s, 1);
+      mbar_init(free_e0 + 8 * s, 1);
+      mbar_init(free_l0 + 8 * s, 1);
+    }
     fence_barrier_init();
   }
   if (warp == 0) tmem_alloc(smem_u32(tmem_slot), TMEM_COLS);
@@ -178,7 +193,7 @@
   }
   const size_t x_off = ((size_t)b * (a.LXP / 8) + x0 / 8) * GROUP_BYTES;
   const size_t y_batch = (size_t)b * (a.LYP / 8) * GROUP_BYTES;
-  if (a.prefetch && tid == 32 * 5) {
+  if (tid == 32 * 5) {
     const size_t e0 = ((size_t)b * a.LX + x0) * a.d, ne = (size_t)min(ROWS, a.LX - x0) * a.d;
     if (IS_PT) {
       l2_prefetch(a.t_feat + e0, ne * 4);
@@ -225,89 +240,142 @@
   tc_fence_after();
   const uint32_t tmem = __shfl_sync(0xffffffffu, *tmem_slot, 0);
 
-  auto issue_stage = [&](int t) {
-    const int s = t % STAGES;
-    const uint32_t bar = bar_full0 + 8 * s;
-    const uint32_t dst = smem_u32(St + s * STAGE_BYTES);
-    const size_t off = y_batch + (size_t)t * Y_PART;
-    mbar_expect_tx(bar, STAGE_BYTES, leader);
-#pragma unroll
-    for (int p = 0; p < NY; ++p)
-      tma_bulk_g2s(dst + p * Y_PART, reinterpret_cast<const char*>(a.y_ops[p]) + off, Y_PART, bar, leader);
+  const bool tracing = a.trace != nullptr && b == 0 && xblk == 0;
+  constexpr int TRACE_TILES = 60;
+  auto stamp = [&](int slot) {
+    if (tracing && (tid == 0 || tid == MMA_WARP * 32)) a.trace[slot] = clock64();
   };
+  auto stamp_tile = [&](int base, int t) {
+    if (t < TRACE_TILES) stamp(base + t);
+  };
+  stamp(0);
+
   if (warp_u == TMA_WARP) {
     mbar_expect_tx(bar_x, NX * X_BYTES, leader);
 #pragma unroll
     for (int p = 0; p < NX; ++p)
       tma_bulk_g2s(smem_u32(Xs + p * X_BYTES), reinterpret_cast<const char*>(a.x_ops[p]) + x_off, X_BYTES, bar_x, leader);
-    for (int t = 0; t < STAGES && t < nty; ++t) issue_stage(t);
-  }
-
-  const float bias2 = a.bias[0] * LOG2E;
-  const int gx = x0 + row;
-  bool valid_x = false, open_x = false;
-  float n1 = 0.f, d1 = 0.f;
-  if (owner) {
-    const ulonglong2 xw = *reinterpret_cast<const ulonglong2*>(a.x_words + ((size_t)b * (a.LXP / 64) + gx / 64) * 2);
-    valid_x = (xw.x >> (gx & 63)) & 1ull;
-    open_x = (xw.y >> (gx & 63)) & 1ull;
-    if (!IS_PT && valid_x) {
-      n1 = a.norm_x[(size_t)b * a.LX + gx] * LOG2E;
-      d1 = a.dlt_x[(size_t)b * a.LX + gx];
-    }
-  }
-  const uint32_t lane_base = tmem + ((uint32_t)(wq * 32) << 16);
-  uint32_t mma_phase = 0;
-  float rsum = 0.f;
-  constexpr uint32_t IDESC_S = idesc_bf16(TY, 0, MMA_M), IDESC_PV = idesc_bf16(DPAD, 1, MMA_M);
-  const uint32_t xs_lo = desc_lo(smem_u32(Xs), 128), ts_lo = desc_lo(smem_u32(Ts), TILE_LBO);
-
-  const bool tracing = a.trace != nullptr && b == 0 && xblk == 0 && tid == MMA_WARP * 32;
-  int ntrace = 0;
-  auto stamp = [&]() {
-    if (tracing && ntrace < 250) a.trace[ntrace++] = clock64();
-  };
-  stamp();
-  if (warp_u == MMA_WARP) mbar_wait(bar_x, 0);
-  stamp();
-  for (int t = 0; t < nty; ++t) {
-    const int s = t % STAGES;
-    const uint32_t st_addr = smem_u32(St + s * STAGE_BYTES);
-    if (warp_u == MMA_WARP) {
-      mbar_wait(bar_full0 + 8 * s, (t / STAGES) & 1);
-      stamp();
+#pragma unroll 1
+    for (int t = 0; t < nty; ++t) {
+      const int s = t % STAGES, k = t / STAGES;
+      const uint32_t dst = smem_u32(St + s * STAGE_BYTES);
+      const size_t off = y_batch + (size_t)t * Y_PART;
+#pragma unroll
+      for (int part = 0; part < 2; ++part) {
+        const uint32_t full = (part ? full_l0 : full_e0) + 8 * s;
+        if (k > 0) mbar_wait((part ? free_l0 : free_e0) + 8 * s, (k - 1) & 1);
+        mbar_expect_tx(full, (part ? N_LATE : NY - N_LATE) * Y_PART, leader);
+#pragma unroll
+        for (int p = 0; p < NY; ++p)
+          if (((LATE >> p) & 1u) == (uint32_t)part)
+            tma_bulk_g2s(dst + p * Y_PART, reinterpret_cast<const char*>(a.y_ops[p]) + off, Y_PART, full, leader);
+      }
+    }
+    if (!IS_PT) {
+      mbar_wait(bar_done, 0);
+      const size_t e0 = ((size_t)b * a.LX + x0) * a.d;
+      const uint32_t bytes = (uint32_t)(min(ROWS, a.LX - x0) * a.d * 4);
+      mbar_expect_tx(bar_rows, 2 * bytes, leader);
+      tma_bulk_g2s(smem_u32(St), a.x_feat + e0, bytes, bar_rows, leader);
+      tma_bulk_g2s(smem_u32(St) + ROWS * a.d * 4, a.dx + e0, bytes, bar_rows, leader);
+    }
+  } else if (warp_u == MMA_WARP) {
+    constexpr uint32_t IDESC_S = idesc_bf16(TY, 0, MMA_M), IDESC_PV = idesc_bf16(DPAD, 1, MMA_M);
+    const uint32_t xs_lo = desc_lo(smem_u32(Xs), 128);
+    mbar_wait(bar_x, 0);
+    auto first_product = [&](int p, uint32_t st_lo) {
+      const int col = p == 0 ? COL_S : p == 1 ? COL_GA : p == 3 ? COL_GB : (MODE == DC ? COL_GA : COL_GB);
+      const bool fresh = p == 0 || p == 1 || (p == 2 && MODE == DQ) || (p == 3 && MODE == DC);
+#pragma unroll
+      for (int k = 0; k < DPAD / 16; ++k)
+        umma_bf16_lh(tmem + col, xs_lo + (p * X_BYTES + k * 256) / 16, desc_hi(GROUP_BYTES),
+                     st_lo + (p * Y_PART + k * 256) / 16, desc_hi(GROUP_BYTES), IDESC_S, !(fresh && k == 0), leader);
+    };
+    auto second_products = [&](int u) {
+      const int s = u % STAGES;
+      if (IS_PT) mbar_wait(full_l0 + 8 * s, (u / STAGES) & 1);
       tc_fence_after();
-      const uint32_t st_lo = desc_lo(st_addr, 128);
-      constexpr int NPROD = IS_PT ? 1 : 4;
-#pragma unroll
-      for (int p = 0; p < NPROD; ++p) {
-        const int col = p == 0 ? COL_S : p == 1 ? COL_GA : p == 3 ? COL_GB : (MODE == DC ? COL_GA : COL_GB);
-        const bool fresh = p == 0 || p == 1 || (p == 2 && MODE == DQ) || (p == 3 && MODE == DC);
-#pragma unroll
-        for (int k = 0; k < DPAD / 16; ++k)
-          umma_bf16_lh(tmem + col, xs_lo + (p * X_BYTES + k * 256) / 16, desc_hi(GROUP_BYTES),
-                       st_lo + (p * Y_PART + k * 256) / 16, desc_hi(GROUP_BYTES), IDESC_S, !(fresh && k == 0), leader);
-      }
-      umma_commit(bar_mma, leader);
-      stamp();
-    }
-    const ulonglong2 words = *reinterpret_cast<const ulonglong2*>(a.y_words + ((size_t)b * (a.LYP / 64) + (t >> 1)) * 2);
-    const int sh = (t & 1) * 32 + half * HALF;
-    const uint32_t wvalid = (uint32_t)(words.x >> sh) & 0xffffu, wopen = (uint32_t)(words.y >> sh) & 0xffffu;
-    if (t + 1 < nty) fetch_ycol(t + 1);
-    if (warp_u == TMA_WARP && t >= 1 && t - 1 + STAGES < nty) {
-      mbar_wait(bar_free0 + 8 * ((t - 1) % STAGES), ((t - 1) / STAGES) & 1);
-      issue_stage(t - 1 + STAGES);
-    }
-    mbar_wait(bar_mma, mma_phase);
-    mma_phase ^= 1;
-    tc_fence_after();
-    stamp();
-
-    {
+      const uint32_t v_lo = desc_lo(smem_u32(St + s * STAGE_BYTES), GROUP_BYTES);
+      const uint32_t ts_lo = desc_lo(smem_u32(Ts + (u & 1) * NT * TILE_BYTES), TILE_LBO);
+#pragma unroll
+      for (int k = 0; k < TY / 16; ++k)
+        umma_bf16_lh(tmem + COL_ACC0, ts_lo + k * 2 * TILE_LBO / 16, desc_hi(128),
+                     v_lo + ((IS_PT ? 1 : 0) * Y_PART + k * 2 * GROUP_BYTES) / 16, desc_hi(128), IDESC_PV, (u > 0) || (k > 0),
+                     leader);
+      if (MODE != DQ) {
+#pragma unroll
+        for (int k = 0; k < TY / 16; ++k)
+          umma_bf16_lh(tmem + COL_ACC1, ts_lo + ((IS_PT ? 0 : TILE_BYTES) + k * 2 * TILE_LBO) / 16, desc_hi(128),
+                       v_lo + ((IS_PT ? 2 : 3) * Y_PART + k * 2 * GROUP_BYTES) / 16, desc_hi(128), IDESC_PV,
+                       (u > 0) || (k > 0), leader);
+      }
+      umma_commit(u == nty - 1 ? bar_done : free_l0 + 8 * s, leader);
+      stamp_tile(192, u);
+    };
+#pragma unroll 1
+    for (int t = 0; t <= nty; ++t) {
+      if (t < nty) {
+        const int s = t % STAGES;
+        const uint32_t ph = (t / STAGES) & 1;
+        const uint32_t st_lo = desc_lo(smem_u32(St + s * STAGE_BYTES), 128);
+        if (t > 0) mbar_wait(bar_s_empty, (t - 1) & 1);
+        mbar_wait(full_e0 + 8 * s, ph);
+        tc_fence_after();
+#pragma unroll
+        for (int p = 0; p < NPROD; ++p)
+          if (!((LATE >> p) & 1u)) first_product(p, st_lo);
+        if (LATE & ((1u << NPROD) - 1u)) {
+          mbar_wait(full_l0 + 8 * s, ph);
+          tc_fence_after();
+#pragma unroll
+          for (int p = 0; p < NPROD; ++p)
+            if ((LATE >> p) & 1u) first_product(p, st_lo);
+        }
+        umma_commit(bar_s_full, leader);
+        umma_commit(free_e0 + 8 * s, leader);
+        stamp_tile(128, t);
+      }
+      if (t > 0) {
+        mbar_wait(bar_ts_full0 + 8 * ((t - 1) & 1), ((t - 1) >> 1) & 1);
+        second_products(t - 1);
+      }
+    }
+  } else if (ew) {
+    const float bias2 = a.bias[0] * LOG2E;
+    const int gx = x0 + row;
+    bool valid_x = false, open_x = false;
+    float n1 = 0.f, d1 = 0.f;
+    if (owner) {
+      const ulonglong2 xw = *reinterpret_cast<const ulonglong2*>(a.x_words + ((size_t)b * (a.LXP / 64) + gx / 64) * 2);
+      valid_x = (xw.x >> (gx & 63)) & 1ull;
+      open_x = (xw.y >> (gx & 63)) & 1ull;
+      if (!IS_PT && valid_x) {
+        n1 = a.norm_x[(size_t)b * a.LX + gx] * LOG2E;
+        d1 = a.dlt_x[(size_t)b * a.LX + gx];
+      }
+    }
+    const uint32_t lane_base = tmem + ((uint32_t)(wq * 32) << 16);
+    float rsum = 0.f;
+#pragma unroll 1
+    for (int t = 0; t < nty; ++t) {
+      const ulonglong2 words = *reinterpret_cast<const ulonglong2*>(a.y_words + ((size_t)b * (a.LYP / 64) + (t >> 1)) * 2);
+      const int sh = (t & 1) * 32 + half * HALF;
+      const uint32_t wvalid = (uint32_t)(words.x >> sh) & 0xffffu, wopen = (uint32_t)(words.y >> sh) & 0xffffu;
+      if (t + 1 < nty) fetch_ycol(t + 1);
+      mbar_wait(bar_s_full, t & 1);
+      tc_fence_after();
+      stamp_tile(1, t);
+      float sv[HALF], ga[HALF], gb[HALF];
+      tmem_ld16(lane_base + COL_S + half * HALF, sv);
+      if (!IS_PT) {
+        tmem_ld16(lane_base + COL_GA + half * HALF, ga);
+        tmem_ld16(lane_base + COL_GB + half * HALF, gb);
+      }
+      tc_fence_before();
+      __syncwarp();
+      if (lane == 0) mbar_arrive(bar_s_empty);
+
       const float* yc = ycol + (t & 1) * 3 * TY + half * HALF;
-      float sv[HALF];
-      tmem_ld16(lane_base + COL_S + half * HALF, sv);
       uint32_t pk0[HALF / 2], pk1[HALF / 2];
       if (IS_PT) {
         float n2[HALF];
@@ -327,9 +395,7 @@
           pk0[c / 2] = *reinterpret_cast<const uint32_t*>(&v);
         }
       } else {
-        float ga[HALF], gb[HALF], n2[HALF], d2[HALF];
-        tmem_ld16(lane_base + COL_GA + half * HALF, ga);
-        tmem_ld16(lane_base + COL_GB + half * HALF, gb);
+        float n2[HALF], d2[HALF];
 #pragma unroll
         for (int c = 0; c < HALF; c += 4) {
           *reinterpret_cast<float4*>(n2 + c) = *reinterpret_cast<const float4*>(yc + c);
@@ -380,7 +446,7 @@
           }
         }
       }
-      unsigned char* trow = Ts + row * 16 + (half * (HALF / 8)) * TILE_LBO;
+      unsigned char* trow = Ts + (t & 1) * NT * TILE_BYTES + row * 16 + (half * (HALF / 8)) * TILE_LBO;
       if (owner) {
 #pragma unroll
         for (int c8 = 0; c8 < HALF / 8; ++c8) {
@@ -390,193 +456,185 @@
                 make_uint4(pk1[c8 * 4], pk1[c8 * 4 + 1], pk1[c8 * 4 + 2], pk1[c8 * 4 + 3]);
         }
       }
-    }
-    if (t + 1 < nty) store_ycol(t + 1);
-    fence_proxy_async();
-    tc_fence_before();
-    __syncthreads();
-    stamp();
-    if (warp_u == MMA_WARP) {
-      tc_fence_after();
-      const uint32_t v_lo = desc_lo(st_addr, GROUP_BYTES);
-#pragma unroll
-      for (int k = 0; k < TY / 16; ++k)
-        umma_bf16_lh(tmem + COL_ACC0, ts_lo + k * 2 * TILE_LBO / 16, desc_hi(128),
-                     v_lo + ((IS_PT ? 1 : 0) * Y_PART + k * 2 * GROUP_BYTES) / 16, desc_hi(128), IDESC_PV, (t > 0) || (k > 0),
-                     leader);
-      if (MODE != DQ) {
-#pragma unroll
-        for (int k = 0; k < TY / 16; ++k)
-          umma_bf16_lh(tmem + COL_ACC1, ts_lo + ((IS_PT ? 0 : TILE_BYTES) + k * 2 * TILE_LBO) / 16, desc_hi(128),
-                       v_lo + ((IS_PT ? 2 : 3) * Y_PART + k * 2 * GROUP_BYTES) / 16, desc_hi(128), IDESC_PV,
-                       (t > 0) || (k > 0), leader);
-      }
-      umma_commit(t == nty - 1 ? bar_mma : bar_free0 + 8 * s, leader);
-    }
-  }
-  mbar_wait(bar_mma, mma_phase);
-  tc_fence_after();
-  __syncthreads();
-  stamp();
-
-  float* stg = reinterpret_cast<float*>(smem);
-  const int d = a.d, dv4 = d >> 2;
-  auto drain = [&](int col0, float* dst) {
+      if (t + 1 < nty) store_ycol(t + 1);
+      fence_proxy_async();
+      named_bar_sync(1, NTHREADS);
+      if (tid == 0) mbar_arrive(bar_ts_full0 + 8 * (t & 1));
+      stamp_tile(64, t);
+    }
+
+    mbar_wait(bar_done, 0);
+    tc_fence_after();
+    named_bar_sync(1, NTHREADS);
+    stamp(250);
+
+    float* stg = reinterpret_cast<float*>(smem);
+    const int d = a.d, dv4 = d >> 2;
+    auto drain = [&](int col0, float* dst) {
 #pragma unroll 1
-    for (int q = half; q < DPAD / 16; q += 2) {
-      float o[16];
-      tmem_ld16(lane_base + col0 + q * 16, o);
-      if (owner) {
-#pragma unroll
-        for (int i = 0; i < 16; i += 4)
-          if (q * 16 + i < STG_STRIDE)
-            *reinterpret_cast<float4*>(dst + row * STG_STRIDE + q * 16 + i) = make_float4(o[i], o[i + 1], o[i + 2], o[i + 3]);
-      }
-    }
-  };
-  if (IS_PT) {
-    drain(COL_ACC0, stg);
-    __syncthreads();
-    for (int i = tid; i < ROWS * dv4; i += NTHREADS) {
-      const int r = i / dv4, c4 = i - r * dv4;
-      if (x0 + r < a.LX)
-        *reinterpret_cast<float4*>(a.dx + ((size_t)b * a.LX + x0 + r) * d + c4 * 4) =
-            *reinterpret_cast<const float4*>(stg + r * STG_STRIDE + c4 * 4);
-    }
-    __syncthreads();
-    drain(COL_ACC1, stg);
-    __syncthreads();
-    char* tp = reinterpret_cast<char*>(a.dt_pack) + x_off;
-    for (int i = tid; i < ROWS * CHUNKS; i += NTHREADS) {
-      const int g8 = i / (CHUNKS * 8), rem = i - g8 * CHUNKS * 8, ch = rem >> 3, r8 = rem & 7;
-      const int r = g8 * 8 + r8;
-      __nv_bfloat162 v[4];
-#pragma unroll
-      for (int e = 0; e < 4; ++e) {
-        const int col = ch * 8 + 2 * e;
-        const bool ok = (x0 + r < a.LX) && col < d;
-        v[e] = __floats2bfloat162_rn(ok ? stg[r * STG_STRIDE + col] : 0.f, ok ? stg[r * STG_STRIDE + col + 1] : 0.f);
-      }
-      *reinterpret_cast<uint4*>(tp + (size_t)i * 16) = *reinterpret_cast<uint4*>(v);
-    }
-    constexpr int NW = NTHREADS / 32, RB = 8;
+      for (int q = half; q < DPAD / 16; q += 2) {
+        float o[16];
+        tmem_ld16(lane_base + col0 + q * 16, o);
+        if (owner) {
+#pragma unroll
+          for (int i = 0; i < 16; i += 4)
+            if (q * 16 + i < STG_STRIDE)
+              *reinterpret_cast<float4*>(dst + row * STG_STRIDE + q * 16 + i) = make_float4(o[i], o[i + 1], o[i + 2], o[i + 3]);
+        }
+      }
+    };
+    if (IS_PT) {
+      drain(COL_ACC0, stg);
+      named_bar_sync(1, NTHREADS);
+      stamp(252);
+      for (int i = tid; i < ROWS * dv4; i += NTHREADS) {
+        const int r = i / dv4, c4 = i - r * dv4;
+        if (x0 + r < a.LX)
+          *reinterpret_cast<float4*>(a.dx + ((size_t)b * a.LX + x0 + r) * d + c4 * 4) =
+              *reinterpret_cast<const float4*>(stg + r * STG_STRIDE + c4 * 4);
+      }
+      named_bar_sync(1, NTHREADS);
+      drain(COL_ACC1, stg);
+      named_bar_sync(1, NTHREADS);
+      stamp(253);
+      char* tp = reinterpret_cast<char*>(a.dt_pack) + x_off;
+      for (int i = tid; i < ROWS * CHUNKS; i += NTHREADS) {
+        const int g8 = i / (CHUNKS * 8), rem = i - g8 * CHUNKS * 8, ch = rem >> 3, r8 = rem & 7;
+        const int r = g8 * 8 + r8;
+        __nv_bfloat162 v[4];
+#pragma unroll
+        for (int e = 0; e < 4; ++e) {
+          const int col = ch * 8 + 2 * e;
+          const bool ok = (x0 + r < a.LX) && col < d;
+          v[e] = __floats2bfloat162_rn(ok ? stg[r * STG_STRIDE + col] : 0.f, ok ? stg[r * STG_STRIDE + col + 1] : 0.f);
+        }
+        *reinterpret_cast<uint4*>(tp + (size_t)i * 16) = *reinterpret_cast<uint4*>(v);
+      }
+      constexpr int NW = NTHREADS / 32, RB = 8;
 #pragma unroll 1
-    for (int r0 = warp; r0 < ROWS; r0 += NW * RB) {
-      float4 tv[RB][2];
-#pragma unroll
-      for (int u = 0; u < RB; ++u) {
-        const int r = r0 + u * NW;
-        const float* trow = a.t_feat + ((size_t)b * a.LX + min(x0 + r, a.LX - 1)) * d;
-#pragma unroll
-        for (int h = 0; h < 2; ++h) {
-          const int c4 = lane + 32 * h;
-          tv[u][h] = c4 < dv4 ? __ldg(reinterpret_cast<const float4*>(trow + c4 * 4)) : make_float4(0.f, 0.f, 0.f, 0.f);
-        }
-      }
-#pragma unroll
-      for (int u = 0; u < RB; ++u) {
-        const int r = r0 + u * NW;
-        float dot = 0.f;
-#pragma unroll
-        for (int h = 0; h < 2; ++h) {
-          const int c4 = lane + 32 * h;
-          if (c4 < dv4) {
-            const float4 sv4 = *reinterpret_cast<const float4*>(stg + r * STG_STRIDE + c4 * 4);
-            dot += tv[u][h].x * sv4.x + tv[u][h].y * sv4.y + tv[u][h].z * sv4.z + tv[u][h].w * sv4.w;
+      for (int r0 = warp; r0 < ROWS; r0 += NW * RB) {
+        float4 tv[RB][2];
+#pragma unroll
+        for (int u = 0; u < RB; ++u) {
+          const int r = r0 + u * NW;
+          const float* trow = a.t_feat + ((size_t)b * a.LX + min(x0 + r, a.LX - 1)) * d;
+#pragma unroll
+          for (int h = 0; h < 2; ++h) {
+            const int c4 = lane + 32 * h;
+            tv[u][h] = c4 < dv4 ? __ldg(reinterpret_cast<const float4*>(trow + c4 * 4)) : make_float4(0.f, 0.f, 0.f, 0.f);
           }
         }
-        dot = warp_sum(dot);
-        if (lane == 0 && x0 + r < a.LX) a.d_col[(size_t)b * a.LX + x0 + r] = dot;
-      }
-    }
-  } else {
-    float* stg1 = stg + ROWS * STG_STRIDE;
-    float* xsum = ycol;
-    static_assert(IS_PT || 2 * ROWS <= 2 * 3 * TY, "xsum fits in ycol");
-    drain(COL_ACC0, stg);
-    if (MODE == DC) drain(COL_ACC1, stg1);
-    if (owner) xsum[half * ROWS + row] = rsum;
-    __syncthreads();
-    const int ngrp = NTHREADS / dv4, rg = tid / dv4, c4 = tid - rg * dv4;
-    const int nrow = min(ROWS, a.LX - x0);
-    float* red = reinterpret_cast<float*>(St);
-    float pt[4] = {0.f, 0.f, 0.f, 0.f}, pf[4] = {0.f, 0.f, 0.f, 0.f}, p_sum = 0.f;
-    if (rg < ngrp) {
-      float wtv[4], wfv[4];
-#pragma unroll
-      for (int e = 0; e < 4; ++e) {
-        wtv[e] = a.w_term[c4 * 4 + e];
-        wfv[e] = a.w_fold ? a.w_fold[c4 * 4 + e] : 1.f;
-      }
-      constexpr int BATCH = 7;
+#pragma unroll
+        for (int u = 0; u < RB; ++u) {
+          const int r = r0 + u * NW;
+          float dot = 0.f;
+#pragma unroll
+          for (int h = 0; h < 2; ++h) {
+            const int c4 = lane + 32 * h;
+            if (c4 < dv4) {
+              const float4 sv4 = *reinterpret_cast<const float4*>(stg + r * STG_STRIDE + c4 * 4);
+              dot += tv[u][h].x * sv4.x + tv[u][h].y * sv4.y + tv[u][h].z * sv4.z + tv[u][h].w * sv4.w;
+            }
+          }
+          dot = warp_sum(dot);
+          if (lane == 0 && x0 + r < a.LX) a.d_col[(size_t)b * a.LX + x0 + r] = dot;
+        }
+      }
+    } else {
+      float* stg1 = stg + ROWS * STG_STRIDE;
+      float* xsum = ycol;
+      static_assert(IS_PT || 2 * ROWS <= 2 * 3 * TY, "xsum fits in ycol");
+      drain(COL_ACC0, stg);
+      if (MODE == DC) drain(COL_ACC1, stg1);
+      if (owner) xsum[half * ROWS + row] = rsum;
+      named_bar_sync(1, NTHREADS);
+      stamp(252);
+      const int ngrp = NTHREADS / dv4, rg = tid / dv4, c4 = tid - rg * dv4;
+      const int nrow = min(ROWS, a.LX - x0);
+      const float* x_rows = reinterpret_cast<const float*>(St);
+      const float* dx_rows = x_rows + ROWS * d;
+      float* red = stg + 2 * ROWS * STG_STRIDE;
+      static_assert(IS_PT || 2 * ROWS * STG_STRIDE * 4 + 8704 <= NX * X_BYTES + 2 * NT * TILE_BYTES, "red fits before St");
+      mbar_wait(bar_rows, 0);
+      float pt[4] = {0.f, 0.f, 0.f, 0.f}, pf[4] = {0.f, 0.f, 0.f, 0.f}, p_sum = 0.f;
+      if (rg < ngrp) {
+        float wtv[4], wfv[4];
+#pragma unroll
+        for (int e = 0; e < 4; ++e) {
+          wtv[e] = a.w_term[c4 * 4 + e];
+          wfv[e] = a.w_fold ? a.w_fold[c4 * 4 + e] : 1.f;
+        }
+        constexpr int BATCH = 7;
 #pragma unroll 1
-      for (int r0 = rg; r0 < nrow; r0 += BATCH * ngrp) {
-        float4 xv[BATCH], dv[BATCH];
-        uchar4 kv[BATCH];
-#pragma unroll
-        for (int u = 0; u < BATCH; ++u) {
-          const int r = r0 + u * ngrp;
-          if (r < nrow) {
-            const size_t gi = ((size_t)b * a.LX + x0 + r) * d + c4 * 4;
-            xv[u] = __ldg(reinterpret_cast<const float4*>(a.x_feat + gi));
-            dv[u] = *reinterpret_cast<const float4*>(a.dx + gi);
-            kv[u] = a.x_keep ? __ldg(reinterpret_cast<const uchar4*>(a.x_keep + gi)) : make_uchar4(1, 1, 1, 1);
+        for (int r0 = rg; r0 < nrow; r0 += BATCH * ngrp) {
+          float4 xv[BATCH], dv[BATCH];
+          uchar4 kv[BATCH];
+#pragma unroll
+          for (int u = 0; u < BATCH; ++u) {
+            const int r = r0 + u * ngrp;
+            if (r < nrow) {
+              const size_t gi = ((size_t)b * a.LX + x0 + r) * d + c4 * 4;
+              xv[u] = *reinterpret_cast<const float4*>(x_rows + r * d + c4 * 4);
+              dv[u] = *reinterpret_cast<const float4*>(dx_rows + r * d + c4 * 4);
+              kv[u] = a.x_keep ? __ldg(reinterpret_cast<const uchar4*>(a.x_keep + gi)) : make_uchar4(1, 1, 1, 1);
+            }
           }
-        }
-#pragma unroll
-        for (int u = 0; u < BATCH; ++u) {
-          const int r = r0 + u * ngrp;
-          if (r < nrow) {
-            const float rs = xsum[r] + xsum[ROWS + r];
-            const float4 v04 = *reinterpret_cast<const float4*>(stg + r * STG_STRIDE + c4 * 4);
-            float4 v14 = make_float4(0.f, 0.f, 0.f, 0.f);
-            if (MODE == DC) v14 = *reinterpret_cast<const float4*>(stg1 + r * STG_STRIDE + c4 * 4);
-            const float x[4] = {xv[u].x, xv[u].y, xv[u].z, xv[u].w}, v0[4] = {v04.x, v04.y, v04.z, v04.w};
-            const float v1[4] = {v14.x, v14.y, v14.z, v14.w};
-            const unsigned char kk[4] = {kv[u].x, kv[u].y, kv[u].z, kv[u].w};
-            float o[4] = {dv[u].x, dv[u].y, dv[u].z, dv[u].w};
-#pragma unroll
-            for (int e = 0; e < 4; ++e) {
-              const float ks = a.x_keep ? (kk[e] ? a.keep_scale : 0.f) : 1.f;
-              const float xd = x[e] * ks;
-              o[e] += ks * fmaf(rs, wtv[e], v0[e] * wfv[e]) + v1[e];
-              pt[e] = fmaf(xd, rs, pt[e]);
-              pf[e] = fmaf(xd, v0[e], pf[e]);
+#pragma unroll
+          for (int u = 0; u < BATCH; ++u) {
+            const int r = r0 + u * ngrp;
+            if (r < nrow) {
+              const float rs = xsum[r] + xsum[ROWS + r];
+              const float4 v04 = *reinterpret_cast<const float4*>(stg + r * STG_STRIDE + c4 * 4);
+              float4 v14 = make_float4(0.f, 0.f, 0.f, 0.f);
+              if (MODE == DC) v14 = *reinterpret_cast<const float4*>(stg1 + r * STG_STRIDE + c4 * 4);
+              const float x[4] = {xv[u].x, xv[u].y, xv[u].z, xv[u].w}, v0[4] = {v04.x, v04.y, v04.z, v04.w};
+              const float v1[4] = {v14.x, v14.y, v14.z, v14.w};
+              const unsigned char kk[4] = {kv[u].x, kv[u].y, kv[u].z, kv[u].w};
+              float o[4] = {dv[u].x, dv[u].y, dv[u].z, dv[u].w};
+#pragma unroll
+              for (int e = 0; e < 4; ++e) {
+                const float ks = a.x_keep ? (kk[e] ? a.keep_scale : 0.f) : 1.f;
+                const float xd = x[e] * ks;
+                o[e] += ks * fmaf(rs, wtv[e], v0[e] * wfv[e]) + v1[e];
+                pt[e] = fmaf(xd, rs, pt[e]);
+                pf[e] = fmaf(xd, v0[e], pf[e]);
+              }
+              p_sum += rs;
+              const size_t gi = ((size_t)b * a.LX + x0 + r) * d + c4 * 4;
+              *reinterpret_cast<float4*>(a.dx + gi) = make_float4(o[0], o[1], o[2], o[3]);
             }
-            p_sum += rs;
-            const size_t gi = ((size_t)b * a.LX + x0 + r) * d + c4 * 4;
-            *reinterpret_cast<float4*>(a.dx + gi) = make_float4(o[0], o[1], o[2], o[3]);
           }
         }
-      }
-      *reinterpret_cast<float4*>(red + (rg * 2 + 0) * d + c4 * 4) = make_float4(pt[0], pt[1], pt[2], pt[3]);
-      *reinterpret_cast<float4*>(red + (rg * 2 + 1) * d + c4 * 4) = make_float4(pf[0], pf[1], pf[2], pf[3]);
-      if (c4 == 0) red[ngrp * 2 * d + rg] = p_sum;
-    }
-    __syncthreads();
-    if (tid < d) {
-      float s_term = 0.f, s_fold = 0.f, s_sum = 0.f;
-      for (int g = 0; g < ngrp; ++g) {
-        s_term += red[(g * 2 + 0) * d + tid];
-        s_fold += red[(g * 2 + 1) * d + tid];
-        if (tid == 0) s_sum += red[ngrp * 2 * d + g];
-      }
-      float* part = a.part + ((size_t)b * nxb + xblk) * PART_STRIDE;
-      part[tid] = s_term;
-      part[DPAD + tid] = s_fold;
-      if (tid == 0) part[2 * DPAD] = s_sum;
-    }
+        *reinterpret_cast<float4*>(red + (rg * 2 + 0) * d + c4 * 4) = make_float4(pt[0], pt[1], pt[2], pt[3]);
+        *reinterpret_cast<float4*>(red + (rg * 2 + 1) * d + c4 * 4) = make_float4(pf[0], pf[1], pf[2], pf[3]);
+        if (c4 == 0) red[ngrp * 2 * d + rg] = p_sum;
+      }
+      named_bar_sync(1, NTHREADS);
+      stamp(253);
+      if (tid < d) {
+        float s_term = 0.f, s_fold = 0.f, s_sum = 0.f;
+        for (int g = 0; g < ngrp; ++g) {
+          s_term += red[(g * 2 + 0) * d + tid];
+          s_fold += red[(g * 2 + 1) * d + tid];
+          if (tid == 0) s_sum += red[ngrp * 2 * d + g];
+        }
+        float* part = a.part + ((size_t)b * nxb + xblk) * PART_STRIDE;
+        part[tid] = s_term;
+        part[DPAD + tid] = s_fold;
+        if (tid == 0) part[2 * DPAD] = s_sum;
+      }
+    }
+    stamp(251);
+    if (tracing && tid == 0) a.trace[255] = min(nty, TRACE_TILES);
   }
   tc_fence_before();
   __syncthreads();
-  stamp();
-  if (tracing) a.trace[255] = ntrace;
   if (warp == 0) tmem_dealloc(tmem, TMEM_COLS);
   if (IS_PT && ready && tid == 0) signal_counter(ready + b);
 }
 
 template <int MODE>
-__global__ void __launch_bounds__(NTHREADS, 1) bidaf_bwd_tc_kernel(const BwdArgs a) {
+__global__ void __launch_bounds__(CTA_THREADS, 1) bidaf_bwd_tc_kernel(const BwdArgs a) {
   bwd_block<MODE>(a, blockIdx.y, blockIdx.x, gridDim.x, nullptr, 0);
 }
 
@@ -588,7 +646,7 @@
   int dq_first;
 };
 
-__global__ void __launch_bounds__(NTHREADS, 1) bidaf_bwd_fused_kernel(const BwdFusedArgs f) {
+__global__ void __launch_bounds__(CTA_THREADS, 1) bidaf_bwd_fused_kernel(const BwdFusedArgs f) {
   const int blk = blockIdx.x;
   if (blk < f.n_pt) {
     bwd_block<PT>(f.k[PT], blk / f.nb[PT], blk % f.nb[PT], f.nb[PT], f.ready, 0);
@@ -612,8 +670,9 @@
   constexpr int ROWS = MODE == PT ? 128 : 64;
   constexpr int NX = MODE == PT ? 1 : 4, NY = MODE == PT ? 3 : 4;
   constexpr int STAGES = MODE == PT ? 3 : 2;
-  return (size_t)NX * (ROWS / 8 * GROUP_BYTES) + 2 * (ROWS * TY * 2) + (size_t)STAGES * NY * Y_PART + 2 * 3 * TY * 4 +
-         (2 + 2 * MAX_STAGES) * 8 + 16;
+  constexpr int NT = MODE == DC ? 2 : 1;
+  return (size_t)NX * (ROWS / 8 * GROUP_BYTES) + 2 * NT * (ROWS * TY * 2) + (size_t)STAGES * NY * Y_PART + 2 * 3 * TY * 4 +
+         NBARS * 8 + 16;
 }
 
 struct ReduceArgs {
@@ -750,33 +809,30 @@
     a.LX = Lq; a.LXP = LqP; a.LY = Lc; a.LYP = LcP; a.d = d;
     a.trace = tracing ? w.trace + 512 : nullptr;
   }
-  static const char* pf_env = getenv("MMB_BIDAF_BWD_PREFETCH");
-  pt.prefetch = dc.prefetch = dq.prefetch = pf_env ? atoi(pf_env) : 1;
   constexpr size_t smem_pt = bwd_smem_bytes<PT>(), smem_dc = bwd_smem_bytes<DC>(), smem_dq = bwd_smem_bytes<DQ>();
   static_assert(smem_dc <= 227 * 1024 && smem_dq <= 227 * 1024 && smem_pt <= 227 * 1024, "shared memory");
   if (!env) {
     constexpr size_t smem = smem_dc > smem_pt ? (smem_dc > smem_dq ? smem_dc : smem_dq) : (smem_pt > smem_dq ? smem_pt : smem_dq);
-    static const char* ord_env = getenv("MMB_BIDAF_BWD_ORDER");
-    const int dq_first = ord_env ? atoi(ord_env) : (Lc >= Lq ? 1 : 0);
+    const int dq_first = Lc >= Lq ? 1 : 0;
     BwdFusedArgs f{{pt, dc, dq}, w.ready, B * (LqP / 128), B * (LcP / 64), B * (LqP / 64), {LqP / 128, LcP / 64, LqP / 64}, dq_first};
     MMB_CUDA(cudaMemsetAsync(w.ready, 0, sizeof(int) * (size_t)B, stream));
     MMB_CUDA(cudaFuncSetAttribute(bidaf_bwd_fused_kernel, cudaFuncAttributeMaxDynamicSharedMemorySize, (int)smem));
-    bidaf_bwd_fused_kernel<<<f.n_pt + f.n_dc + f.n_dq, NTHREADS, smem, stream>>>(f);
+    bidaf_bwd_fused_kernel<<<f.n_pt + f.n_dc + f.n_dq, CTA_THREADS, smem, stream>>>(f);
     if (int rc = check_launch("bidaf_bwd_fused_kernel")) return rc;
   } else {
     if (stages & 2) {
       MMB_CUDA(cudaFuncSetAttribute(bidaf_bwd_tc_kernel<PT>, cudaFuncAttributeMaxDynamicSharedMemorySize, (int)smem_pt));
-      bidaf_bwd_tc_kernel<PT><<<dim3(LqP / 128, B), NTHREADS, smem_pt, stream>>>(pt);
+      bidaf_bwd_tc_kernel<PT><<<dim3(LqP / 128, B), CTA_THREADS, smem_pt, stream>>>(pt);
       if (int rc = check_launch("bidaf_bwd_tc_kernel<PT>")) return rc;
     }
     if (stages & 4) {
       MMB_CUDA(cudaFuncSetAttribute(bidaf_bwd_tc_kernel<DC>, cudaFuncAttributeMaxDynamicSharedMemorySize, (int)smem_dc));
-      bidaf_bwd_tc_kernel<DC><<<dim3(LcP / 64, B), NTHREADS, smem_dc, stream>>>(dc);
+      bidaf_bwd_tc_kernel<DC><<<dim3(LcP / 64, B), CTA_THREADS, smem_dc, stream>>>(dc);
       if (int rc = check_launch("bidaf_bwd_tc_kernel<DC>")) return rc;
     }
     if (stages & 8) {
       MMB_CUDA(cudaFuncSetAttribute(bidaf_bwd_tc_kernel<DQ>, cudaFuncAttributeMaxDynamicSharedMemorySize, (int)smem_dq));
-      bidaf_bwd_tc_kernel<DQ><<<dim3(LqP / 64, B), NTHREADS, smem_dq, stream>>>(dq);
+      bidaf_bwd_tc_kernel<DQ><<<dim3(LqP / 64, B), CTA_THREADS, smem_dq, stream>>>(dq);
       if (int rc = check_launch("bidaf_bwd_tc_kernel<DQ>")) return rc;
     }
   }
diff --git a/mmbidaf_b200/csrc/bidaf_fwd_tc5.cu b/mmbidaf_b200/csrc/bidaf_fwd_tc5.cu
--- a/mmbidaf_b200/csrc/bidaf_fwd_tc5.cu
+++ b/mmbidaf_b200/csrc/bidaf_fwd_tc5.cu
@@ -61,12 +61,6 @@
   }
 };
 
-__device__ __forceinline__ void mbar_arrive(uint32_t bar) {
-  asm volatile("mbarrier.arrive.shared::cta.b64 _, [%0];" ::"r"(bar) : "memory");
-}
-__device__ __forceinline__ void named_bar_sync(int id, int nthreads) {
-  asm volatile("bar.sync %0, %1;" ::"r"(id), "r"(nthreads) : "memory");
-}
 __device__ __forceinline__ void tmem_ld16_nowait(uint32_t taddr, uint32_t* r) {
   asm volatile(
       "tcgen05.ld.sync.aligned.32x32b.x16.b32 {%0,%1,%2,%3,%4,%5,%6,%7,%8,%9,%10,%11,%12,%13,%14,%15}, [%16];"
diff --git a/mmbidaf_b200/csrc/tc_common.cuh b/mmbidaf_b200/csrc/tc_common.cuh
--- a/mmbidaf_b200/csrc/tc_common.cuh
+++ b/mmbidaf_b200/csrc/tc_common.cuh
@@ -54,6 +54,12 @@
     if (done) return;
   }
   __trap();
+}
+__device__ __forceinline__ void mbar_arrive(uint32_t bar) {
+  asm volatile("mbarrier.arrive.shared::cta.b64 _, [%0];" ::"r"(bar) : "memory");
+}
+__device__ __forceinline__ void named_bar_sync(int id, int nthreads) {
+  asm volatile("bar.sync %0, %1;" ::"r"(id), "r"(nthreads) : "memory");
 }
 __device__ __forceinline__ void tma_bulk_g2s(uint32_t dst, const void* src, uint32_t bytes, uint32_t bar, uint32_t leader) {
   asm volatile(
```
